# santi-pdp/segan_pytorch

Measured on AMD Instinct MI355X. Metric: 16384-sample waveform chunks/sec (GAN step), higher is better.
Workload: dtype f32

## Files before the change

segan_pytorch_amd/_lib.py:

```python
import ctypes
import os
import re
from ctypes import POINTER, Structure, c_char_p, c_double, c_float, c_int, c_int32, c_int64, c_size_t, c_void_p

_HERE = os.path.dirname(os.path.abspath(__file__))
LIB_PATH = os.environ.get('SEGAN_HIP_LIB') or os.path.join(_HERE, 'libsegan_hip.so')
HEADER_PATH = os.path.join(os.path.dirname(_HERE), 'include', 'segan_hip.h')


class SeganSrc(Structure):
    _fields_ = [('p0', c_void_p), ('p1', c_void_p), ('C0', c_int32), ('C1', c_int32),
                ('scale', c_void_p), ('shift', c_void_p), ('slope', c_void_p)]


_SCALARS = {'int': c_int, 'float': c_float, 'double': c_double, 'size_t': c_size_t,
            'int64_t': c_int64, 'long long': c_int64}


class _Defines(dict):

    def __init__(self, where):
        dict.__init__(self)
        self.where, self.unread = where, {}

    def __missing__(self, name):
        raise RuntimeError('{}: no integer `#define {}` ({})'.format(
            self.where, name, self.unread.get(name, 'not defined')))


def _ctype(text, decl, ret=False):
    tok = [w for w in re.findall(r'\w+|\S', text) if w != 'const']
    if not ret:
        if len(tok) < 2 or not re.match(r'[A-Za-z_]\w*$', tok[-1]):
            raise RuntimeError('unnamed or unreadable argument `{}` in `{}`'.format(text.strip(), decl))
        tok.pop()
    stars = tok.count('*')
    base = tok[:len(tok) - stars]
    if stars and base and '*' not in base:
        if not ret:
            return POINTER(SeganSrc) if tok == ['segan_src', '*'] else c_void_p
        if tok == ['char', '*']:
            return c_char_p
    elif ret and tok == ['void']:
        return None
    elif ' '.join(tok) in _SCALARS:
        return _SCALARS[' '.join(tok)]
    raise RuntimeError('unknown type `{}` in `{}`'.format(text.strip(), decl))


def read_header(text, where='<text>'):
    text = re.sub(r'/\*.*?\*/|//[^\n]*', ' ', text, flags=re.S)
    defines = _Defines(where)
    seen = {}
    for name, val in re.findall(r'^[ \t]*#[ \t]*define[ \t]+(SEGAN_\w+)[ \t]+(\S.*?)[ \t]*$', text, flags=re.M):
        seen.setdefault(name, []).append(val)
    for name, vals in seen.items():
        if len(set(vals)) == 1 and re.match(r'-?(0[xX][0-9a-fA-F]+|[1-9]\d*|0)$', vals[0]):
            defines[name] = int(vals[0], 0)
        else:
            defines.unread[name] = ' / '.join('#define {} {}'.format(name, v) for v in vals)
    text = re.sub(r'^[ \t]*#.*$', '', text, flags=re.M)
    signatures = {}
    for m in re.finditer(r'[^;{}]*\bsegan_\w+\s*\([^;]*(;|$)', text):
        decl = ' '.join(m.group().split())
        d = re.match(r'([\w\s*]+?)\s*\b(segan_\w+)\s*\(([^()]*)\)\s*;$', decl)
        if not d or d.group(2) in signatures:
            raise RuntimeError('{}: cannot read the declaration `{}`'.format(where, decl))
        args = [] if d.group(3).strip() == 'void' else d.group(3).split(',')
        signatures[d.group(2)] = (_ctype(d.group(1), decl, ret=True), [_ctype(a, decl) for a in args])
    return signatures, defines


def _read_header_file():
    if not os.path.exists(HEADER_PATH):
        raise RuntimeError('segan_pytorch_amd: {} not found. The ctypes binding is read from the '
                           'header the library is built against.'.format(HEADER_PATH))
    with open(HEADER_PATH) as f:
        return read_header(f.read(), HEADER_PATH)


SIGNATURES, DEFINES = _read_header_file()

PAD_REFLECT = DEFINES['SEGAN_PAD_REFLECT']
PAD_ZERO = DEFINES['SEGAN_PAD_ZERO']
ACT_NONE = DEFINES['SEGAN_ACT_NONE']
ACT_TANH = DEFINES['SEGAN_ACT_TANH']
ABI_VERSION = DEFINES['SEGAN_ABI_VERSION']

_lib = None


def load():
    global _lib
    if _lib is not None:
        return _lib
    if not os.path.exists(LIB_PATH):
        raise RuntimeError(
            'segan_pytorch_amd: {} not found. Build it with `make` (or '
            '`python -c "import __graft_entry__ as g; g.build()"`) at the repo root. '
            'There is no non-HIP fallback.'.format(LIB_PATH))
    try:
        import torch
        if torch.cuda.is_available():
            torch.cuda.init()
    except ImportError:
        pass
    lib = ctypes.CDLL(LIB_PATH)
    for name, (res, args) in SIGNATURES.items():
        fn = getattr(lib, name)
        fn.restype = res
        fn.argtypes = args
    ver = lib.segan_abi_version()
    if ver != ABI_VERSION:
        raise RuntimeError('libsegan_hip ABI {} != expected {}'.format(ver, ABI_VERSION))
    _lib = lib
    return lib


def check(rc, what=''):
    if rc != 0:
        msg = load().segan_last_error()
        raise RuntimeError('libsegan_hip {} failed ({}): {}'.format(
            what, rc, msg.decode() if msg else '?'))
```

segan_pytorch_amd/csrc/segan_conv.hip:

```cpp
#include "segan_conv_tile.h"


struct TileWork {
  int tile, c0, c1;
  bool partial;
  int piece;
};

struct TileIter {
  int tileA;
  long unit, unit_end;
  int first_tile;
  __device__ __forceinline__ void init(const CorrArgs& a, int nch) {
    tileA = blockIdx.x;
    unit = (long)blockIdx.x * a.sk_units;
    unit_end = min(unit + (long)a.sk_units, a.sk_total);
    first_tile = (int)(unit / nch);
  }
  __device__ __forceinline__ bool next(const CorrArgs& a, int nch, TileWork& w) {
    if (tileA < a.sk_nfull) {
      const int rd = tileA / (int)gridDim.x;
      const int left = a.sk_nfull - rd * (int)gridDim.x;
      w.tile = rd * (int)gridDim.x + xcd_remap(blockIdx.x, left < (int)gridDim.x ? left : (int)gridDim.x);
      w.c0 = 0; w.c1 = nch; w.partial = false; w.piece = 0;
      tileA += gridDim.x;
      return true;
    }
    if (unit < unit_end) {
      const int t = (int)(unit / nch);
      w.c0 = (int)(unit - (long)t * nch);
      w.c1 = min(nch, w.c0 + (int)(unit_end - unit));
      unit += w.c1 - w.c0;
      w.tile = a.sk_nfull + t;
      w.partial = (w.c0 != 0) || (w.c1 != nch);
      w.piece = t - first_tile;
      return true;
    }
    return false;
  }
};

template <int MB, int U, int KC, int NI, int NJ, bool SHIFT, int FMODE = 0, int ZP = -1, int NPT = 32>
__device__ __forceinline__ void corr_mma_chunk(const float* Wl, const float* Il, int RLs,
                                               const int (&aoff)[NI], const int (&boff)[NJ],
                                               const int (&rsh)[NI], f32x16 (&acc)[NI][NJ],
                                               float (&b30)[NJ], int h, const int (&aoffx)[NI],
                                               const int (&boffx)[NJ]) {
  static_assert(FMODE == 0 || (!SHIFT && ZP < 0), "the pair trick of the F form has no row shifts");
  constexpr int NBI = SHIFT ? NI : 1;
  constexpr int CVC = KC / U;
  constexpr bool ZT = ZP >= 0 && CVC >= 2;
  typedef const volatile __attribute__((address_space(3))) float* ldsp;
  auto special = [](int i) { return ZT && (32 * i) / NPT == ZP; };
  auto skipped = [&](int i, int s) { return special(i) && ((2 * s) % U) == 0; };
  float av0[NI], av1[NI], bv0[NBI][NJ], bv1[NBI][NJ];
  auto read_step = [&](int s, float (&av)[NI], float (&bv)[NBI][NJ]) {
    const int kk = 2 * s;
    const int c = kk / U, u = kk % U;
    ldsp wr = (ldsp)(Wl + kk * MB);
    ldsp ir = (ldsp)(Il + c * RLs + u);
#pragma unroll
    for (int i = 0; i < NI; ++i)
      if (!skipped(i, s)) av[i] = wr[aoff[i]];
#pragma unroll
    for (int i = 0; i < NBI; ++i)
#pragma unroll
      for (int j = 0; j < NJ; ++j)
        if (!(SHIFT && skipped(i, s))) bv[i][j] = ir[boff[j] + (SHIFT ? rsh[i] : 0)];
  };
  constexpr int NS = FMODE == 1 ? KC / 2 - 1 : KC / 2;
  auto mma_step = [&](int s, const float (&av)[NI], float (&bv)[NBI][NJ]) {
    if (FMODE == 2 && s == NS - 1) {
#pragma unroll
      for (int j = 0; j < NJ; ++j) bv[0][j] = h ? b30[j] : bv[0][j];
    }
#pragma unroll
    for (int i = 0; i < NI; ++i)
#pragma unroll
      for (int j = 0; j < NJ; ++j)
        if (!skipped(i, s))
          acc[i][j] = __builtin_amdgcn_mfma_f32_32x32x2f32(av[i], bv[SHIFT ? i : 0][j], acc[i][j],
                                                           0, 0, 0);
  };
// ... 920 lines not shown
  SEGAN_REQUIRE(precision_ok(precision), "deconv1d_dgrad: precision must be 0, 1, 3 or 4");
  SEGAN_REQUIRE(stride_ok(S), "deconv1d_dgrad: stride %d not in {1,2,4}", S);
  SEGAN_REQUIRE(K >= 1 && K <= 32, "deconv1d_dgrad: kernel width %d not in [1,32]", K);
  SEGAN_REQUIRE(B > 0 && N > 0 && M > 0 && Ls > 0, "deconv1d_dgrad: bad sizes");
  SEGAN_REQUIRE(M0 >= 0 && M0 <= M, "deconv1d_dgrad: split %d outside [0,%d]", M0, M);
  SEGAN_REQUIRE(dy && wf, "deconv1d_dgrad: NULL pointer");
  SEGAN_REQUIRE(dx0 || dx1, "deconv1d_dgrad: both destinations NULL");
  const int U = 32 / S;
  CorrArgs a = {};
  a.acc_block = acc_block;
  a.in.p0 = dy; a.in.p1 = nullptr; a.in.C0 = N; a.in.C1 = 0;
  a.in.scale = a.in.shift = a.in.slope = nullptr;
  a.wp = (const float*)wf;
  a.bias = nullptr; a.halo = nullptr;
  a.B = B; a.Cv = N * S; a.Ktot = N * 32; a.RP = f_pitch(M); a.Rvalid = M;
  a.Tcols = Ls; a.Ctot = B * Ls;
  a.Lin = S * Ls; a.padL = pad; a.mode = SEGAN_PAD_ZERO; a.roll = 0;
  a.win_start = 0; a.H = U - 1;
  a.NP = 1; a.Nout = 0;
  if (M0 == 0) { a.out0 = dx1; a.OC0 = M; a.out1 = nullptr; a.OC1 = 0; }
  else { a.out0 = dx0; a.OC0 = M0; a.out1 = dx1; a.OC1 = M - M0; }
  a.Lout = Ls; a.act = SEGAN_ACT_NONE;
  a.out0_elems = (size_t)B * a.OC0 * Ls;
  a.out1_elems = (size_t)B * a.OC1 * Ls;
  a.f_pair = f_pair(N, K); a.zphase = -1;
  if (precision) {
    CorrArgs a2 = a;
    const int e = segan_corr_bf2_f(a2, U, wf, precision, scratch, scratch_bytes, (hipStream_t)stream);
    return e;
  }
  set_scratch(a, scratch, scratch_bytes);
  return launch_corr<true, false>(a, U, (hipStream_t)stream);
}

extern "C" int segan_deconv1d_fwd(const segan_src* x, const void* wt, const float* w,
                                  const float* bias, float* y, int B, int M, int N, int Ls, int K,
                                  int S, int pad, int act, int precision, void* scratch,
                                  size_t scratch_bytes, void* stream) {
  const int acc_block = precision == SEGAN_PREC_FP32_BLOCKED;
  if (acc_block) precision = SEGAN_PREC_FP32;
  SEGAN_REQUIRE(precision_ok(precision), "deconv1d_fwd: precision must be 0, 1, 3 or 4");
  SEGAN_REQUIRE(stride_ok(S), "deconv1d_fwd: stride %d not in {1,2,4}", S);
  SEGAN_REQUIRE(K >= 1 && K <= 32, "deconv1d_fwd: kernel width %d not in [1,32]", K);
  SEGAN_REQUIRE(B > 0 && N > 0 && M > 0 && Ls > 0, "deconv1d_fwd: bad sizes");
  SEGAN_REQUIRE(y && (wt || (w && N <= 2)), "deconv1d_fwd: NULL pointer");
  SEGAN_REQUIRE(pad >= 0 && K - 2 * pad - S == (K & 1),
                "deconv1d_fwd: K=%d S=%d pad=%d does not give an output of S*Ls samples", K, S, pad);
  SEGAN_REQUIRE(act == SEGAN_ACT_NONE || act == SEGAN_ACT_TANH, "deconv1d_fwd: bad activation");
  if (int e = check_src(x, M, "deconv1d_fwd")) return e;
  const int U = 32 / S;
  CorrArgs a = {};
  a.acc_block = acc_block;
  a.in = *x;
  a.wp = (const float*)wt;
  a.out0 = y; a.out1 = nullptr; a.bias = bias; a.halo = nullptr;
  a.NP = t_np(N, S); a.Nout = N;
  a.B = B; a.Cv = M; a.Ktot = M * U; a.RP = t_pitch(N, S); a.Rvalid = S * a.NP;
  a.Tcols = Ls; a.Ctot = B * Ls;
  a.Lin = Ls; a.padL = 0; a.mode = SEGAN_PAD_ZERO; a.roll = 0;
  int cmin = 1 << 30, cmax = 0;
  for (int r = 0; r < S; ++r) {
    const int c = (r + pad) / S;
    cmin = c < cmin ? c : cmin;
    cmax = c > cmax ? c : cmax;
  }
  for (int r = 0; r < 4; ++r) a.rowshift[r] = r < S ? (r + pad) / S - cmin : 0;
  a.win_start = cmin - (U - 1);
  a.H = U - 1 + (cmax - cmin);
  a.OC0 = N; a.OC1 = 0; a.Lout = S * Ls; a.act = act;
  a.o_padL = 0; a.o_roll = 0; a.o_padR = 0;
  a.out0_elems = (size_t)B * N * S * Ls;
  a.f_pair = 0; a.zphase = t_zphase(K, S, pad);
  if (w && N <= 2) return segan_launch_tsmall(a, w, K, M, N, S, pad, (hipStream_t)stream);
  if (precision && act == SEGAN_ACT_NONE) {
    CorrArgs a2 = a;
    const int e = segan_corr_bf2_t(a2, U, wt, precision, scratch, scratch_bytes, (hipStream_t)stream);
    return e;
  }
  SEGAN_REQUIRE(precision == 0, "deconv1d_fwd: tanh epilogue only on the fp32 path");
  set_scratch(a, scratch, scratch_bytes);
  return launch_corr<false, true>(a, U, (hipStream_t)stream);
}

extern "C" int segan_conv1d_dgrad(const float* da, const void* wt, const float* w, float* dx,
                                  float* halo, int B, int N, int M, int L, int K, int S, int padL,
                                  int roll, int precision, void* scratch, size_t scratch_bytes,
                                  void* stream) {
  const int acc_block = precision == SEGAN_PREC_FP32_BLOCKED;
  if (acc_block) precision = SEGAN_PREC_FP32;
  SEGAN_REQUIRE(precision_ok(precision), "conv1d_dgrad: precision must be 0, 1, 3 or 4");
  SEGAN_REQUIRE(stride_ok(S), "conv1d_dgrad: stride %d not in {1,2,4}", S);
  SEGAN_REQUIRE(K >= 1 && K <= 32, "conv1d_dgrad: kernel width %d not in [1,32]", K);
  SEGAN_REQUIRE(B > 0 && N > 0 && M > 0 && L > 0 && L % S == 0, "conv1d_dgrad: bad sizes");
  SEGAN_REQUIRE(da && dx && halo && (wt || (w && N <= 2)), "conv1d_dgrad: NULL pointer");
  SEGAN_REQUIRE(roll > -L && roll < L, "conv1d_dgrad: |roll| must be < L");
  const int padR = K - 1 - padL >= 0 ? (K - S - padL > 0 ? K - S - padL : 0) : -1;
  SEGAN_REQUIRE(padL >= 0 && padR >= 0 && padL < L && K - S - padL < L, "conv1d_dgrad: bad padding");
  const int U = 32 / S;
  const int Ls = L / S;
  hipStream_t st = (hipStream_t)stream;
  CorrArgs a = {};
  a.acc_block = acc_block;
  a.in.p0 = da; a.in.p1 = nullptr; a.in.C0 = M; a.in.C1 = 0;
  a.in.scale = a.in.shift = a.in.slope = nullptr;
  a.wp = (const float*)wt;
  a.out0 = dx; a.out1 = nullptr; a.bias = nullptr; a.halo = halo;
  a.NP = t_np(N, S); a.Nout = N;
  a.B = B; a.Cv = M; a.Ktot = M * U; a.RP = t_pitch(N, S); a.Rvalid = S * a.NP;
  a.Tcols = (L + padL + padR - 1) / S + 1;
  a.Ctot = B * a.Tcols;
  a.Lin = Ls; a.padL = 0; a.mode = SEGAN_PAD_ZERO; a.roll = 0;
  for (int r = 0; r < 4; ++r) a.rowshift[r] = 0;
  a.win_start = -(U - 1);
  a.H = U - 1;
  a.OC0 = N; a.OC1 = 0; a.Lout = L; a.act = SEGAN_ACT_NONE;
  a.o_padL = padL; a.o_roll = roll; a.o_padR = padR;
  a.out0_elems = (size_t)B * N * L;
  a.halo_elems = (size_t)B * N * (padL + padR);
  a.f_pair = 0; a.zphase = t_zphase(K, S, 0);
  set_scratch(a, scratch, scratch_bytes);
  int e;
  if (w && N <= 2) {
    e = segan_launch_tsmall(a, w, K, M, N, S, 0, st);
  } else if (precision) {
    CorrArgs a2 = a;
    e = segan_corr_bf2_t(a2, U, wt, precision, scratch, scratch_bytes, st);
  } else {
    e = launch_corr<false, true>(a, U, st);
  }
  if (e) return e;
  if (padL + padR > 0) {
    const int rows = B * N;
    const int per_sample = (padL < L - 1 - padR) ? 1 : 0;
    const long nthreads = per_sample ? (long)rows * (padL + padR) : rows;
    hipLaunchKernelGGL(fold_halo_kernel, dim3((unsigned)((nthreads + 255) / 256)), dim3(256), 0, st,
                       dx, halo, rows, L, padL, padR, roll, per_sample);
    return segan_check_launch("fold_halo_kernel");
  }
  return SEGAN_OK;
}

static bool short_ok(int N, int M, int L, int K, int S, int padL) {
  if (!stride_ok(S) || L % S != 0) return false;
  const int Ls = L / S;
  return (Ls == 4 || Ls == 8 || Ls == 16 || Ls == 32 || Ls == 64) && N % 4 == 0 &&
         M % CS_KC == 0 && K >= 1 && K <= 32 && padL >= 0 && K - 1 - padL >= 0 && padL < L &&
         K - S - padL < L;
}

extern "C" size_t segan_packed_g_bytes(int M, int N, int S) {
  if (!stride_ok(S) || M <= 0 || N <= 0) return 0;
  return (size_t)M * N * 32 * sizeof(float);
}

extern "C" int segan_pack_weights_g(const float* w, float* wg, int M, int N, int K, int S,
                                    void* stream) {
  SEGAN_REQUIRE(w && wg && M > 0 && N > 0, "pack_weights_g: bad arguments");
  SEGAN_REQUIRE(stride_ok(S) && K >= 1 && K <= 32, "pack_weights_g: stride in {1,2,4}, K <= 32");
  const size_t total = (size_t)M * N * 32;
  const int blocks = (int)((total + 255) / 256 > 8192 ? 8192 : (total + 255) / 256);
  hipLaunchKernelGGL(pack_g_kernel, dim3(blocks), dim3(256), 0, (hipStream_t)stream, w, wg, M, N, K,
                     S);
  return segan_check_launch("pack_weights_g");
}

extern "C" int segan_conv1d_dgrad_short(const float* da, const float* wg, float* dx, int B, int N,
                                        int M, int L, int K, int S, int padL, int roll,
                                        void* stream) {
  SEGAN_REQUIRE(da && wg && dx && B > 0, "conv1d_dgrad_short: bad arguments");
  SEGAN_REQUIRE(roll > -L && roll < L, "conv1d_dgrad_short: |roll| must be < L");
  if (!short_ok(N, M, L, K, S, padL)) {
    segan_set_error("conv1d_dgrad_short: geometry not covered (L/S in {4,8,16,32,64}, N %% 4 == 0, "
                    "M %% 16 == 0)");
    return SEGAN_EUNSUPPORTED;
  }
  ShortArgs a;
  a.da = da; a.wg = wg; a.dx = dx;
  a.B = B; a.N = N; a.M = M; a.L = L; a.Ls = L / S; a.padL = padL;
  a.padRw = K - S - padL > 0 ? K - S - padL : 0;
  a.roll = roll;
  a.ncoltiles = ceil_div(B, 128 / a.Ls);
  const size_t lds = 4 * 32 * 65 * sizeof(float);
  const dim3 grid((unsigned)(N / 4 * a.ncoltiles));
  static const bool blocked = [] {
    const char* e = getenv("SEGAN_SHORT_ORDER");
    return !(e && e[0] == '0');
  }();
  a.xr8 = a.xbc = 0;
  if (blocked && (N / 4) % 8 == 0) {
    a.xr8 = N / 4 / 8;
    a.xbc = a.xr8 >= 128 ? 1 : 128 / a.xr8;
  }
  hipStream_t st = (hipStream_t)stream;
  if (S == 4) hipLaunchKernelGGL(conv_dgrad_short_kernel<4>, grid, dim3(256), lds, st, a);
  else if (S == 2) hipLaunchKernelGGL(conv_dgrad_short_kernel<2>, grid, dim3(256), lds, st, a);
  else hipLaunchKernelGGL(conv_dgrad_short_kernel<1>, grid, dim3(256), lds, st, a);
  return segan_check_launch("conv_dgrad_short_kernel");
}
```

segan_pytorch_amd/csrc/segan_conv_edge.hip:

```cpp
#include "segan_conv_shared.h"

template <int S, int N, int PM, int KT>
__global__ __launch_bounds__(256) void tsmall_kernel(const CorrArgs a, const float* __restrict__ w,
                                                     int Krt, int M) {
  const int K = KT ? KT : Krt;
  constexpr int U = 32 / S;
  constexpr int MC = 16;
  constexpr int TW = 256 + U;
  __shared__ float xs[MC][TW + 1];
  const int tid = threadIdx.x;
  const int b = blockIdx.y;
  const int q0 = blockIdx.x * 256;
  const int q = q0 + tid;
  float acc[S][N];
#pragma unroll
  for (int r = 0; r < S; ++r)
#pragma unroll
    for (int n = 0; n < N; ++n) acc[r][n] = 0.0f;

  const int t0 = q0 + a.win_start + tid, t1 = t0 + 256;
  const bool ok0 = t0 >= 0 && t0 < a.Lin, ok1 = tid < U && t1 >= 0 && t1 < a.Lin;
  const int o0 = ok0 ? t0 : 0, o1 = ok1 ? t1 : 0;
  const int bo0 = b * a.in.C0 * a.Lin, bo1 = b * a.in.C1 * a.Lin;
  float pv0[MC], pv1[MC];
  auto load_rows = [&](int mc0) {
#pragma unroll
    for (int mc = 0; mc < MC; ++mc) {
      const int m = mc0 + mc < M ? mc0 + mc : 0;
      const bool seg1 = m >= a.in.C0;
      const float* rowp = seg1 ? a.in.p1 + (size_t)(m - a.in.C0) * a.Lin + bo1
                               : a.in.p0 + (size_t)m * a.Lin + bo0;
      pv0[mc] = rowp[o0];
      pv1[mc] = rowp[o1];
    }
  };
  load_rows(0);
  for (int mc0 = 0; mc0 < M; mc0 += MC) {
#pragma unroll
    for (int mc = 0; mc < MC; ++mc) {
      const bool mok = mc0 + mc < M;
      const ChanXf xf = segan_chan_xf(a.in, mok ? mc0 + mc : 0);
      xs[mc][tid] = (mok && ok0) ? segan_apply_xf(xf, pv0[mc]) : 0.0f;
      if (tid < U) xs[mc][256 + tid] = (mok && ok1) ? segan_apply_xf(xf, pv1[mc]) : 0.0f;
    }
    __syncthreads();
    if (mc0 + MC < M) load_rows(mc0 + MC);
    const int mcn = min(MC, M - mc0);
    for (int mc = 0; mc < mcn; ++mc) {
      float xv[U + 1];
#pragma unroll
      for (int j = 0; j <= U; ++j) xv[j] = xs[mc][tid + j];
      const float* wm = w + (size_t)(mc0 + mc) * N * K;
#pragma unroll
      for (int r = 0; r < S; ++r) {
        const int rho = (r + PM) % S;
        const int cs = (r + PM) / S;
#pragma unroll
        for (int u = 0; u < U; ++u) {
          const int k = S * u + rho;
          if (KT) {
            if (k < KT) {
#pragma unroll
              for (int n = 0; n < N; ++n)
                acc[r][n] = fmaf(wm[n * KT + k], xv[cs + (U - 1) - u], acc[r][n]);
            }
          } else {
            const int kc = k < K ? k : K - 1;
#pragma unroll
            for (int n = 0; n < N; ++n) {
              float wv = wm[n * K + kc];
              wv = k < K ? wv : 0.0f;
              acc[r][n] = fmaf(wv, xv[cs + (U - 1) - u], acc[r][n]);
            }
          }
        }
      }
    }
    __syncthreads();
  }
  if (q >= a.Tcols) return;
#pragma unroll
  for (int r = 0; r < S; ++r)
#pragma unroll
    for (int n = 0; n < N; ++n) {
      float v = acc[r][n] + (a.bias ? a.bias[n] : 0.0f);
      if (a.act == SEGAN_ACT_TANH) v = tanhf(v);
      const int P = S * q + r;
      int ii = P - a.o_padL;
      const size_t rowoff = (size_t)b * N + n;
      if (ii >= 0 && ii < a.Lout) {
        if (a.o_roll != 0) {
          ii -= a.o_roll;
          if (ii < 0) ii += a.Lout;
          if (ii >= a.Lout) ii -= a.Lout;
        }
        a.out0[rowoff * (size_t)a.Lout + ii] = v;
      } else if (a.halo != nullptr) {
        const int hl = a.o_padL + a.o_padR;
        if (ii < 0) a.halo[rowoff * hl + P] = v;
        else if (ii - a.Lout < a.o_padR) a.halo[rowoff * hl + a.o_padL + (ii - a.Lout)] = v;
      }
    }
}

template <int S, int N, int KT>
static int launch_tsmall_snk(const CorrArgs& a, const float* w, int K, int M, int pad,
                             hipStream_t st) {
  dim3 grid(ceil_div(a.Tcols, 256), a.B);
  switch (pad % S) {
    case 0: hipLaunchKernelGGL((tsmall_kernel<S, N, 0, KT>), grid, dim3(256), 0, st, a, w, K, M); break;
    case 1: hipLaunchKernelGGL((tsmall_kernel<S, N, 1 % S, KT>), grid, dim3(256), 0, st, a, w, K, M); break;
    case 2: hipLaunchKernelGGL((tsmall_kernel<S, N, 2 % S, KT>), grid, dim3(256), 0, st, a, w, K, M); break;
    default: hipLaunchKernelGGL((tsmall_kernel<S, N, 3 % S, KT>), grid, dim3(256), 0, st, a, w, K, M); break;
  }
  return segan_check_launch("tsmall_kernel");
}

template <int S, int N>
static int launch_tsmall_sn(const CorrArgs& a, const float* w, int K, int M, int pad,
                            hipStream_t st) {
  if (K == 31) return launch_tsmall_snk<S, N, 31>(a, w, K, M, pad, st);
  return launch_tsmall_snk<S, N, 0>(a, w, K, M, pad, st);
}


template <int N, int PM>
__global__ __launch_bounds__(256) void tsmall4_kernel(const CorrArgs a, const float* __restrict__ w,
                                                      int M) {
  constexpr int S = 4, U = 8, KT = 31, Q = 4;
  constexpr int MC = 8;
  constexpr int TWQ = Q * 256 + 12;
  __shared__ __attribute__((aligned(16))) float xs[MC][TWQ];
  const int tid = threadIdx.x;
  const int b = blockIdx.y;
  const int q0 = blockIdx.x * (Q * 256);
  typedef float f32x2 __attribute__((ext_vector_type(2)));
  f32x2 acc[Q / 2][S][N];
#pragma unroll
  for (int i = 0; i < Q / 2; ++i)
#pragma unroll
    for (int r = 0; r < S; ++r)
#pragma unroll
      for (int n = 0; n < N; ++n) acc[i][r][n] = f32x2{0.0f, 0.0f};
  int so[5];
  unsigned sok = 0u;
#pragma unroll
  for (int i = 0; i < 5; ++i) {
    const int j = tid + 256 * i;
    const int t = q0 + a.win_start + j;
    const bool ok = (i < 4 || tid < 12) && t >= 0 && t < a.Lin;
    so[i] = ok ? t : 0;
    if (ok) sok |= 1u << i;
  }
  const int bo0 = b * a.in.C0 * a.Lin, bo1 = b * a.in.C1 * a.Lin;
  float pv[MC][5];
  auto load_rows = [&](int mc0) {
#pragma unroll
    for (int mc = 0; mc < MC; ++mc) {
      const int m = mc0 + mc < M ? mc0 + mc : 0;
      const bool seg1 = m >= a.in.C0;
      const float* rowp = seg1 ? a.in.p1 + (size_t)(m - a.in.C0) * a.Lin + bo1
                               : a.in.p0 + (size_t)m * a.Lin + bo0;
#pragma unroll
      for (int i = 0; i < 5; ++i) pv[mc][i] = rowp[so[i]];
    }
  };
  load_rows(0);
  for (int mc0 = 0; mc0 < M; mc0 += MC) {
#pragma unroll
    for (int mc = 0; mc < MC; ++mc) {
      const bool mok = mc0 + mc < M;
      const ChanXf xf = segan_chan_xf(a.in, mok ? mc0 + mc : 0);
#pragma unroll
      for (int i = 0; i < 4; ++i)
        xs[mc][tid + 256 * i] = (mok && ((sok >> i) & 1u)) ? segan_apply_xf(xf, pv[mc][i]) : 0.0f;
      if (tid < 12) xs[mc][1024 + tid] = (mok && ((sok >> 4) & 1u)) ? segan_apply_xf(xf, pv[mc][4]) : 0.0f;
    }
    __syncthreads();
    if (mc0 + MC < M) load_rows(mc0 + MC);
    const int mcn = min(MC, M - mc0);
    for (int mc = 0; mc < mcn; ++mc) {
      f32x2 xe[6], xo[5];
#pragma unroll
      for (int i = 0; i < 3; ++i) {
        const f32x4 t4 = *reinterpret_cast<const f32x4*>(&xs[mc][4 * tid + 4 * i]);
        xe[2 * i] = f32x2{t4[0], t4[1]};
        xe[2 * i + 1] = f32x2{t4[2], t4[3]};
      }
#pragma unroll
      for (int i = 0; i < 5; ++i) xo[i] = f32x2{xs[mc][4 * tid + 2 * i + 1], xs[mc][4 * tid + 2 * i + 2]};
      typedef const __attribute__((address_space(4))) float cfl;
      constexpr int NPW = (N * KT + 1) / 2;
      cfl* wm = (cfl*)w + (size_t)(mc0 + mc) * N * KT;
      f32x2 wp[NPW];
#pragma unroll
      for (int p = 0; p < NPW; ++p) {
        const int f0 = 2 * p + 1 < N * KT ? 2 * p : N * KT - 2;
        wp[p] = f32x2{wm[f0], wm[f0 + 1]};
      }
#pragma unroll
      for (int r = 0; r < S; ++r) {
        const int rho = (r + PM) % S, cs = (r + PM) / S;
#pragma unroll
        for (int u = 0; u < U; ++u) {
          const int k = S * u + rho;
          if (k < KT) {
#pragma unroll
            for (int n = 0; n < N; ++n) {
              const int f = n * KT + k;
              const bool last = 2 * (f >> 1) + 1 >= N * KT;
              const int p = f >> 1, h = last ? 1 : (f & 1);
#pragma unroll
              for (int ip = 0; ip < Q / 2; ++ip) {
                const int j = 2 * ip + cs + (U - 1) - u;
                const f32x2 xp = (j & 1) ? xo[j >> 1] : xe[j >> 1];
                if (h)
                  asm("v_pk_fma_f32 %0, %1, %2, %0 op_sel:[1,0,0] op_sel_hi:[1,1,1]"
                      : "+v"(acc[ip][r][n]) : "s"(wp[p]), "v"(xp));
                else
                  asm("v_pk_fma_f32 %0, %1, %2, %0 op_sel:[0,0,0] op_sel_hi:[0,1,1]"
                      : "+v"(acc[ip][r][n]) : "s"(wp[p]), "v"(xp));
              }
            }
          }
        }
      }
    }
    __syncthreads();
  }
#pragma unroll
  for (int n = 0; n < N; ++n) {
    const float bs = a.bias ? a.bias[n] : 0.0f;
    const size_t rowoff = (size_t)b * N + n;
#pragma unroll
    for (int i = 0; i < Q; ++i) {
      const int q = q0 + Q * tid + i;
      if (q >= a.Tcols) continue;
      float v[S];
#pragma unroll
      for (int r = 0; r < S; ++r) {
        v[r] = acc[i >> 1][r][n][i & 1] + bs;
        if (a.act == SEGAN_ACT_TANH) v[r] = tanhf(v[r]);
      }
      const int i0 = S * q - a.o_padL;
      if (a.o_roll == 0 && i0 >= 0 && i0 + 3 < a.Lout && (a.o_padL & 3) == 0) {
        const f32x4 o = {v[0], v[1], v[2], v[3]};
        *reinterpret_cast<f32x4*>(a.out0 + rowoff * (size_t)a.Lout + i0) = o;
        continue;
      }
#pragma unroll
      for (int r = 0; r < S; ++r) {
        const int P = S * q + r;
        int ii = P - a.o_padL;
        if (ii >= 0 && ii < a.Lout) {
          if (a.o_roll != 0) {
            ii -= a.o_roll;
            if (ii < 0) ii += a.Lout;
            if (ii >= a.Lout) ii -= a.Lout;
          }
          a.out0[rowoff * (size_t)a.Lout + ii] = v[r];
        } else if (a.halo != nullptr) {
          const int hl = a.o_padL + a.o_padR;
          if (ii < 0) a.halo[rowoff * hl + P] = v[r];
          else if (ii - a.Lout < a.o_padR) a.halo[rowoff * hl + a.o_padL + (ii - a.Lout)] = v[r];
        }
      }
    }
  }
}

template <int N>
static int launch_tsmall4(const CorrArgs& a, const float* w, int M, int pad, hipStream_t st) {
  dim3 grid(ceil_div(a.Tcols, 1024), a.B);
  switch (pad % 4) {
    case 0: hipLaunchKernelGGL((tsmall4_kernel<N, 0>), grid, dim3(256), 0, st, a, w, M); break;
    case 1: hipLaunchKernelGGL((tsmall4_kernel<N, 1>), grid, dim3(256), 0, st, a, w, M); break;
    case 2: hipLaunchKernelGGL((tsmall4_kernel<N, 2>), grid, dim3(256), 0, st, a, w, M); break;
    default: hipLaunchKernelGGL((tsmall4_kernel<N, 3>), grid, dim3(256), 0, st, a, w, M); break;
  }
  return segan_check_launch("tsmall4_kernel");
}

int segan_launch_tsmall(CorrArgs& a, const float* w, int K, int M, int N, int S, int pad,
                         hipStream_t st) {
  if (int e = segan_src_defaults(&a.in, st, "tsmall")) return e;
  if (S == 4 && K == 31 && a.Tcols >= 1024)
    return N == 1 ? launch_tsmall4<1>(a, w, M, pad, st) : launch_tsmall4<2>(a, w, M, pad, st);
  if (N == 1) {
    if (S == 4) return launch_tsmall_sn<4, 1>(a, w, K, M, pad, st);
    if (S == 2) return launch_tsmall_sn<2, 1>(a, w, K, M, pad, st);
    return launch_tsmall_sn<1, 1>(a, w, K, M, pad, st);
  }
  if (S == 4) return launch_tsmall_sn<4, 2>(a, w, K, M, pad, st);
  if (S == 2) return launch_tsmall_sn<2, 2>(a, w, K, M, pad, st);
  return launch_tsmall_sn<1, 2>(a, w, K, M, pad, st);
}


template <int S, int N, int XW>
__device__ __forceinline__ void fsmall_stage_window(const CorrArgs& a, int b, int t0, int tid,
                                                    float (&xs)[N][XW]) {
  constexpr int NX = (XW + 255) / 256;
  constexpr int BT = 6;
  const float* rows[N];
  ChanXf xf[N];
#pragma unroll
  for (int n = 0; n < N; ++n) {
    rows[n] = segan_src_row(a.in, b, n, a.Lin);
    xf[n] = segan_chan_xf(a.in, n);
  }
#pragma unroll
  for (int g0 = 0; g0 < NX; g0 += BT) {
    float v[N][BT];
    int idx[BT];
#pragma unroll
    for (int i = 0; i < BT; ++i) {
      const int j = tid + 256 * (g0 + i);
      idx[i] = (g0 + i < NX && j < XW) ? segan_hi_index(S * t0 + j, a.Lin, a.padL, a.mode, a.roll) : -1;
#pragma unroll
      for (int n = 0; n < N; ++n) v[n][i] = rows[n][idx[i] >= 0 ? idx[i] : 0];
    }
#pragma unroll
    for (int i = 0; i < BT; ++i) {
      const int j = tid + 256 * (g0 + i);
      if (g0 + i < NX && j < XW) {
#pragma unroll
        for (int n = 0; n < N; ++n) xs[n][j] = idx[i] >= 0 ? segan_apply_xf(xf[n], v[n][i]) : 0.0f;
      }
    }
  }
}

template <int S, int N, int WST>
__device__ __forceinline__ void fsmall_stage_weights(const CorrArgs& a, int m0, int tid, float* ws) {
  constexpr int U = 32 / S;
  constexpr int NW = 64 * N * 32 / 256;
  constexpr int BT = 8;
  static_assert(NW % BT == 0, "weight staging batches");
#pragma unroll
  for (int g0 = 0; g0 < NW; g0 += BT) {
    float v[BT];
#pragma unroll
    for (int i = 0; i < BT; ++i) {
      const int e = tid + 256 * (g0 + i);
      const int ml = e & 63, nk = e >> 6;
      const int n = nk >> 5, k = nk & 31;
      const int row = (n * S + k % S) * U + k / S;
      const int m = m0 + ml;
      v[i] = a.wp[(size_t)row * a.RP + (m < a.RP ? m : 0)];
      v[i] = m < a.RP ? v[i] : 0.0f;
    }
#pragma unroll
    for (int i = 0; i < BT; ++i) {
      const int e = tid + 256 * (g0 + i);
      const int ml = e & 63, nk = e >> 6;
      ws[ml * WST + (nk >> 5) * 32 + (nk & 31)] = v[i];
    }
  }
}

template <int S, int N>
__global__ __launch_bounds__(256) void fsmall_kernel(const CorrArgs a, int M) {
  constexpr int XW = S * 256 + 32;
  constexpr int WST = N * 32 + 4;
  __shared__ __attribute__((aligned(16))) float xs[N][XW];
  __shared__ __attribute__((aligned(16))) float ws[64 * WST];
  const int tid = threadIdx.x;
  const int b = blockIdx.y;
  const int t0 = blockIdx.x * 256;
  fsmall_stage_window<S, N, XW>(a, b, t0, tid, xs);
  const int t = t0 + tid;
  for (int m0 = 0; m0 < M; m0 += 64) {
    fsmall_stage_weights<S, N, WST>(a, m0, tid, ws);
    __syncthreads();
    float xv[N][32];
#pragma unroll
    for (int n = 0; n < N; ++n) {
      if (S == 4) {
#pragma unroll
        for (int i = 0; i < 8; ++i) {
// ... 144 lines not shown
```

segan_pytorch_amd/csrc/segan_conv_shared.h:

```cpp
#pragma once
#include "segan_common.h"
#include <stdlib.h>

#define KCH 64

struct ColTile {
  int col0, b0, t_first, len0;
};

__device__ __forceinline__ ColTile make_coltile(int col0, int Tcols, int NBcols) {
  ColTile t;
  t.col0 = col0;
  t.b0 = col0 / Tcols;
  t.t_first = col0 - t.b0 * Tcols;
  t.len0 = min(Tcols - t.t_first, NBcols);
  return t;
}

__device__ __forceinline__ void lds_pos_decode(const ColTile& ct, int j, int Tcols, int H, int& s,
                                               int& tau) {
  if (j < ct.len0 + H) {
    s = 0;
    tau = ct.t_first + j;
  } else {
// ... 62 lines not shown
  int Ctot;
  int cols_per_split;
  int H, RLw;
  int ls_magic;
  int per_magic;
  int bf_qc;
  int bf_cps;
  int Mp;
  int w2_cps, w2_nch;
  int w2_cpsample;
  int w2_spc;
  int w2_lsshift;
  int w2_pw, w2_nld;
  float* w2_slabs;
};

__device__ __forceinline__ float epi_bias(const float* bias, int base, int rl0, int h) {
  typedef const __attribute__((address_space(4))) float cfloat;
  cfloat* bp = (cfloat*)bias + base;
  const float lo = bp[rl0], hi = bp[rl0 + 4];
  return h ? hi : lo;
}

__device__ __forceinline__ void split3b(float x, __bf16& p1, __bf16& p2, __bf16& p3) {
  p1 = (__bf16)x;
  const float r1 = x - (float)p1;
  p2 = (__bf16)r1;
  const float r2 = r1 - (float)p2;
  p3 = (__bf16)r2;
}

static inline int cur_device() {
  int d = 0;
  (void)hipGetDevice(&d);
  return d & 15;
}

template <typename K>
static void allow_big_lds(K kern, bool (&done)[16]) {
  const int d = cur_device();
  if (!done[d]) {
    (void)hipFuncSetAttribute(reinterpret_cast<const void*>(kern),
                              hipFuncAttributeMaxDynamicSharedMemorySize, 160 * 1024);
    done[d] = true;
  }
}

template <typename K>
static int resident_per_cu(K kern, size_t lds, int (&occ)[16], size_t (&occ_lds)[16], int fallback = 2) {
  const int d = cur_device();
  if (occ[d] == 0 || occ_lds[d] != lds) {
    int nb = 0;
    if (hipOccupancyMaxActiveBlocksPerMultiprocessor(&nb, reinterpret_cast<const void*>(kern), 256,
                                                     lds) != hipSuccess || nb < 1)
      nb = fallback;
    occ[d] = nb > 4 ? 4 : nb;
    occ_lds[d] = lds;
  }
  return occ[d];
}

static inline int f_pitch(int M) { return M <= 64 ? 64 : round_up(M, 128); }
static inline int f_rows(int N) { return round_up(N * 32, KCH); }
static inline int t_pitch(int N, int S) { return S * t_np(N, S); }
static inline int t_rows(int M, int S) { return round_up(M * (32 / S), KCH); }

static inline int f_pair(int N, int K) { return K == 31 && N > 2 && (N & 1) == 0; }
static inline int t_zphase(int K, int S, int pad_t) {
  return (K == 31 && S > 1) ? (((S - 1 - pad_t) % S) + S) % S : -1;
}

static inline bool stride_ok(int S) { return S == 1 || S == 2 || S == 4; }
static inline bool precision_ok(int p) { return p == 0 || p == 1 || p == 3; }
static inline int check_src(const segan_src* s, int C, const char* what) {
  SEGAN_REQUIRE(s != nullptr && s->p0 != nullptr, "%s: source is NULL", what);
  SEGAN_REQUIRE(s->C0 > 0 && s->C1 >= 0 && s->C0 + s->C1 == C,
                "%s: channel segments %d+%d != %d", what, s->C0, s->C1, C);
  SEGAN_REQUIRE(s->C1 == 0 || s->p1 != nullptr, "%s: second segment pointer is NULL", what);
  return SEGAN_OK;
}

int segan_launch_tsmall(CorrArgs& a, const float* w, int K, int M, int N, int S, int pad, hipStream_t st);
int segan_launch_fsmall(CorrArgs& a, int M, int N, int S, hipStream_t st);

void segan_note_corr_launch(int kind, unsigned grid, const CorrArgs& a, int ntiles);
int segan_corr_bf2_f(CorrArgs& a, int U, const void* wp3, int planes, void* scratch,
                     size_t scratch_bytes, hipStream_t st);
int segan_corr_bf2_t(CorrArgs& a, int U, const void* wp3, int planes, void* scratch,
                     size_t scratch_bytes, hipStream_t st);
size_t segan_corr_bf2_scratch_bytes(int B, int Cv, int Tcols, int H, int planes);
int segan_wgrad_bf2(WgradArgs& a, int U, int planes, void* scratch, size_t scratch_bytes, hipStream_t st);
void segan_note_wgrad_launch(int kind, int tiles, int nsplit, int chunks_per_split);
size_t segan_wgrad_bf2_scratch_bytes(int B, int M, int N, int Ls, int S, int planes);
```

segan_pytorch_amd/csrc/segan_pointwise.hip:

```cpp
#include "segan_common.h"

#define PW_THREADS 256

static int pw_nsplit(int B, int C, int L) {
  int ns = ceil_div(2048, C);
  if (ns > B) ns = B;
  long per = (long)B * L / ns;
  while (ns > 1 && per < 2048) {
    ns = (ns + 1) / 2;
    per = (long)B * L / ns;
  }
  return ns < 1 ? 1 : ns;
}

extern "C" int segan_bn_nsplit(int B, int C, int L) {
  if (B <= 0 || C <= 0 || L <= 0) return 0;
  return pw_nsplit(B, C, L);
}

template <int NV>
__device__ __forceinline__ void block_sum(float (&v)[NV], float* sm) {
  const int lane = threadIdx.x & 63, wave = threadIdx.x >> 6;
#pragma unroll
  for (int k = 0; k < NV; ++k) v[k] = warp_sum(v[k]);
  if (lane == 0)
#pragma unroll
    for (int k = 0; k < NV; ++k) sm[wave * NV + k] = v[k];
  __syncthreads();
  if (threadIdx.x == 0) {
#pragma unroll
    for (int k = 0; k < NV; ++k) {
      float s = 0.f;
      for (int w = 0; w < PW_THREADS / 64; ++w) s += sm[w * NV + k];
      v[k] = s;
    }
  }
  __syncthreads();
}

struct ChanRange {
  int c, b_beg, b_end;
};
__device__ __forceinline__ ChanRange chan_range(int B, int nsplit) {
  ChanRange r;
  r.c = blockIdx.x;
  const int per = (B + nsplit - 1) / nsplit;
  r.b_beg = blockIdx.y * per;
  r.b_end = min(B, r.b_beg + per);
  return r;
}

__device__ __forceinline__ void chan_combine(float& n, float& mean, float& m2, float nb, float mb,
                                             float qb) {
  const float tot = n + nb;
  if (tot <= 0.0f) return;
  const float d = mb - mean;
  const float f = nb / tot;
  mean = fmaf(d, f, mean);
  m2 = m2 + qb + d * d * n * f;
  n = tot;
}

__global__ void bn_partial_kernel(const float* __restrict__ x, float* __restrict__ ws, int B, int C,
                                  int L, int nsplit) {
  __shared__ float sm[3 * (PW_THREADS / 64)];
  const ChanRange cr = chan_range(B, nsplit);
  const int nb = cr.b_end - cr.b_beg;
  const float* base = x + ((size_t)cr.b_beg * C + cr.c) * L;
  const size_t sstride = (size_t)C * L;
  const bool vec = (L & 3) == 0 && ((uintptr_t)x & 15) == 0;
  const int Lv = vec ? L >> 2 : L;
  int tr = PW_THREADS;
  while (tr > Lv && tr > 1) tr >>= 1;
  const int rp = PW_THREADS / tr;
  const int t0 = threadIdx.x % tr, r0 = threadIdx.x / tr;
  float K = 0.0f, s1 = 0.0f, s2 = 0.0f, n = 0.0f;
  if (r0 < nb && t0 < Lv) K = base[(size_t)r0 * sstride + (vec ? 4 * t0 : t0)];
  for (int b = r0; b < nb; b += rp) {
    const float* row = base + b * sstride;
    if (vec) {
      for (int t = t0; t < Lv; t += tr) {
        const f32x4 u = *reinterpret_cast<const f32x4*>(row + 4 * t);
#pragma unroll
        for (int e = 0; e < 4; ++e) {
          const float d = u[e] - K;
          s1 += d;
          s2 = fmaf(d, d, s2);
        }
        n += 4.0f;
      }
    } else {
      for (int t = t0; t < Lv; t += tr) {
        const float d = row[t] - K;
        s1 += d;
        s2 = fmaf(d, d, s2);
        n += 1.0f;
      }
    }
  }
  float mean = 0.0f, m2 = 0.0f;
  if (n > 0.0f) {
    const float r = s1 / n;
    mean = K + r;
    m2 = fmaxf(s2 - s1 * r, 0.0f);
  }
#pragma unroll
  for (int o = 32; o > 0; o >>= 1) {
    const float nb2 = __shfl_down(n, o, 64), mb2 = __shfl_down(mean, o, 64), qb2 = __shfl_down(m2, o, 64);
    chan_combine(n, mean, m2, nb2, mb2, qb2);
  }
  const int lane = threadIdx.x & 63, wave = threadIdx.x >> 6;
  if (lane == 0) {
    sm[3 * wave] = n; sm[3 * wave + 1] = mean; sm[3 * wave + 2] = m2;
  }
  __syncthreads();
  if (threadIdx.x == 0) {
    for (int w = 1; w < PW_THREADS / 64; ++w) chan_combine(n, mean, m2, sm[3 * w], sm[3 * w + 1], sm[3 * w + 2]);
    float* w = ws + ((size_t)blockIdx.y * C + cr.c) * 3;
    w[0] = n;
    w[1] = mean;
    w[2] = m2;
  }
}

__device__ __forceinline__ void bn_affine(float gamma, float beta, float mean, float rstd,
                                          float& scale, float& shift) {
  scale = gamma * rstd;
  shift = fmaf(-mean, scale, beta);
}

__global__ void bn_final_kernel(const float* __restrict__ ws, const float* gamma, const float* beta,
                                float eps, float momentum, float* running_mean, float* running_var,
                                float* mean_o, float* rstd_o, float* scale_o, float* shift_o, int C,
                                int nsplit) {
  const int c = blockIdx.x * blockDim.x + threadIdx.x;
  if (c >= C) return;
  double n = 0.0, mean = 0.0, m2 = 0.0;
  for (int s = 0; s < nsplit; ++s) {
    const float* w = ws + ((size_t)s * C + c) * 3;
    const double nb = w[0], mb = w[1], qb = w[2];
    if (nb <= 0.0) continue;
    const double tot = n + nb;
    const double d = mb - mean;
    mean += d * nb / tot;
    m2 += qb + d * d * n * nb / tot;
    n = tot;
  }
  const double var = n > 0 ? m2 / n : 0.0;
  const float rstd = (float)(1.0 / sqrt(var + (double)eps));
  const float g = gamma ? gamma[c] : 1.0f;
  const float bt = beta ? beta[c] : 0.0f;
  float sc, sh;
  bn_affine(g, bt, (float)mean, rstd, sc, sh);
  if (mean_o) mean_o[c] = (float)mean;
  if (rstd_o) rstd_o[c] = rstd;
  if (scale_o) scale_o[c] = sc;
  if (shift_o) shift_o[c] = sh;
  if (running_mean) running_mean[c] = (1.0f - momentum) * running_mean[c] + momentum * (float)mean;
  if (running_var) {
    const double unb = n > 1 ? m2 / (n - 1.0) : var;
    running_var[c] = (1.0f - momentum) * running_var[c] + momentum * (float)unb;
  }
}

extern "C" int segan_bn_stats(const float* x, const float* gamma, const float* beta, float eps,
                              float momentum, float* running_mean, float* running_var, float* mean,
                              float* rstd, float* scale, float* shift, float* ws, int B, int C,
                              int L, void* stream) {
  SEGAN_REQUIRE(x && ws, "bn_stats: NULL pointer");
  SEGAN_REQUIRE(B > 0 && C > 0 && L > 0, "bn_stats: bad sizes");
  hipStream_t st = (hipStream_t)stream;
  const int ns = pw_nsplit(B, C, L);
  hipLaunchKernelGGL(bn_partial_kernel, dim3(C, ns), dim3(PW_THREADS), 0, st, x, ws, B, C, L, ns);
  hipLaunchKernelGGL(bn_final_kernel, dim3(ceil_div(C, 64)), dim3(64), 0, st, ws, gamma, beta, eps,
                     momentum, running_mean, running_var, mean, rstd, scale, shift, C, ns);
  return segan_check_launch("bn_stats");
}

extern "C" int segan_bn_partial(const float* x, float* ws, int B, int C, int L, void* stream) {
  SEGAN_REQUIRE(x && ws, "bn_partial: NULL pointer");
  SEGAN_REQUIRE(B > 0 && C > 0 && L > 0, "bn_partial: bad sizes");
  const int ns = pw_nsplit(B, C, L);
  hipLaunchKernelGGL(bn_partial_kernel, dim3(C, ns), dim3(PW_THREADS), 0, (hipStream_t)stream, x, ws,
                     B, C, L, ns);
  return segan_check_launch("bn_partial");
}

extern "C" int segan_bn_final(const float* ws, int nsplit_total, const float* gamma,
                              const float* beta, float eps, float momentum, float* running_mean,
                              float* running_var, float* mean, float* rstd, float* scale,
                              float* shift, int C, void* stream) {
  SEGAN_REQUIRE(ws && nsplit_total > 0 && C > 0, "bn_final: bad arguments");
  hipLaunchKernelGGL(bn_final_kernel, dim3(ceil_div(C, 64)), dim3(64), 0, (hipStream_t)stream, ws,
                     gamma, beta, eps, momentum, running_mean, running_var, mean, rstd, scale, shift,
                     C, nsplit_total);
  return segan_check_launch("bn_final");
}

__global__ void affine_prelu_kernel(const float* __restrict__ x, const float* scale,
                                    const float* shift, const float* slope, float* __restrict__ y,
                                    size_t total, int C, int L) {
  for (size_t i = blockIdx.x * (size_t)blockDim.x + threadIdx.x; i < total;
       i += (size_t)gridDim.x * blockDim.x) {
    const int c = (int)((i / L) % C);
    float v = x[i];
    v = fmaf(v, scale ? scale[c] : 1.0f, shift ? shift[c] : 0.0f);
    if (slope) v = v > 0.f ? v : v * slope[c];
    y[i] = v;
  }
}

extern "C" int segan_affine_prelu(const float* x, const float* scale, const float* shift,
                                  const float* slope, float* y, int B, int C, int L, void* stream) {
// ... 15 lines not shown
    y[i] = tanhf(fmaf(x[i], scale ? scale[c] : 1.0f, shift ? shift[c] : 0.0f));
  }
}

extern "C" int segan_affine_tanh(const float* x, const float* scale, const float* shift, float* y,
                                 int B, int C, int L, void* stream) {
  SEGAN_REQUIRE(x && y, "affine_tanh: NULL pointer");
  SEGAN_REQUIRE(B > 0 && C > 0 && L > 0, "affine_tanh: bad sizes");
  const size_t total = (size_t)B * C * L;
  const int blocks = (int)((total + 255) / 256 > 4096 ? 4096 : (total + 255) / 256);
  hipLaunchKernelGGL(affine_tanh_kernel, dim3(blocks), dim3(256), 0, (hipStream_t)stream, x, scale,
                     shift, y, total, C, L);
  return segan_check_launch("affine_tanh");
}

__global__ void scale_mask_kernel(const float* __restrict__ x, const float* scale,
                                  const float* __restrict__ mask, float* __restrict__ y,
                                  size_t total, int C, int L) {
  for (size_t i = blockIdx.x * (size_t)blockDim.x + threadIdx.x; i < total;
       i += (size_t)gridDim.x * blockDim.x) {
    const int c = (int)((i / L) % C);
    y[i] = x[i] * (scale ? scale[c] : 1.0f) * mask[i];
  }
}

extern "C" int segan_scale_mask(const float* x, const float* scale, const float* mask, float* y,
                                int B, int C, int L, void* stream) {
  SEGAN_REQUIRE(x && mask && y, "scale_mask: NULL pointer");
  SEGAN_REQUIRE(B > 0 && C > 0 && L > 0, "scale_mask: bad sizes");
  const size_t total = (size_t)B * C * L;
  const int blocks = (int)((total + 255) / 256 > 4096 ? 4096 : (total + 255) / 256);
  hipLaunchKernelGGL(scale_mask_kernel, dim3(blocks), dim3(256), 0, (hipStream_t)stream, x, scale,
                     mask, y, total, C, L);
  return segan_check_launch("scale_mask");
}

__global__ void sum_skip_kernel(const float* __restrict__ x0, const float* slope0,
                                const float* __restrict__ x1, const float* alpha,
                                float* __restrict__ out, size_t total, int C, int L) {
  for (size_t i = blockIdx.x * (size_t)blockDim.x + threadIdx.x; i < total;
       i += (size_t)gridDim.x * blockDim.x) {
    const int c = (int)((i / L) % C);
    float v = x0[i];
    if (slope0) v = v > 0.f ? v : v * slope0[c];
    out[i] = fmaf(alpha[c], x1[i], v);
  }
}

extern "C" int segan_sum_skip(const float* x0, const float* slope0, const float* x1,
                              const float* alpha, float* out, int B, int C, int L, void* stream) {
  SEGAN_REQUIRE(x0 && x1 && alpha && out, "sum_skip: NULL pointer");
  SEGAN_REQUIRE(B > 0 && C > 0 && L > 0, "sum_skip: bad sizes");
  const size_t total = (size_t)B * C * L;
  const int blocks = (int)((total + 255) / 256 > 4096 ? 4096 : (total + 255) / 256);
  hipLaunchKernelGGL(sum_skip_kernel, dim3(blocks), dim3(256), 0, (hipStream_t)stream, x0, slope0,
                     x1, alpha, out, total, C, L);
  return segan_check_launch("sum_skip");
}

struct ActBwdArgs {
  const float* a;
  const float* dh;
  const float* dskip;
  const float* slope;
  const float* alpha;
  const float* mean;
  const float* rstd;
  const float* gamma;
  const float* beta;
  float* da;
  float* ws;
  int B, C, L, nsplit;
  float inv_count;
};

template <int PHASE>
__global__ void act_bwd_kernel(const ActBwdArgs p) {
  __shared__ float sm[16];
  const ChanRange cr = chan_range(p.B, p.nsplit);
  const int c = cr.c;
  const int nb = cr.b_end - cr.b_beg;
  const float sl = p.slope ? p.slope[c] : 1.0f;
  const float al = p.alpha ? p.alpha[c] : 0.0f;
  float mu = 0.f, rs = 1.f, ga = 1.f, be = 0.f, dbeta_m = 0.f, dgamma_m = 0.f, sc = 1.f, sh = 0.f;
  if (PHASE != 0) {
    mu = p.mean[c];
    rs = p.rstd[c];
    ga = p.gamma ? p.gamma[c] : 1.0f;
    be = p.beta ? p.beta[c] : 0.0f;
    bn_affine(ga, be, mu, rs, sc, sh);
  }
  if (PHASE == 2) {
    const float* tot = p.ws + (size_t)p.nsplit * p.C * 4 + (size_t)c * 2;
    dbeta_m = tot[0] * p.inv_count;
    dgamma_m = tot[1] * p.inv_count;
  }
  float r[3] = {0.f, 0.f, 0.f};
  const bool has_skip = p.dskip != nullptr;
  auto elem = [&](float av, float dh, float ds) -> float {
    if (PHASE == 0) {
      float g = dh * (av > 0.f ? 1.0f : sl);
      r[0] += dh * (av > 0.f ? 0.0f : av);
      if (has_skip) {
        g = fmaf(al, ds, g);
        r[1] = fmaf(ds, av, r[1]);
      }
      r[2] += g;
      return g;
    }
    const float xh = (av - mu) * rs;
    const float v = fmaf(av, sc, sh);
    const float g = dh * (v > 0.f ? 1.0f : sl);
    if (PHASE == 1) {
      r[0] += dh * (v > 0.f ? 0.0f : v);
      r[1] += g;
      r[2] = fmaf(g, xh, r[2]);
      return 0.0f;
    }
    const float d = ga * rs * (g - dbeta_m - xh * dgamma_m);
    r[0] += d;
    return d;
  };
  const size_t base = ((size_t)cr.b_beg * p.C + c) * p.L;
  const size_t sstride = (size_t)p.C * p.L;
  const bool vec = (p.L & 3) == 0 &&
                   (((uintptr_t)p.a | (uintptr_t)p.dh | (uintptr_t)p.dskip | (uintptr_t)p.da) & 15) == 0;
  const int Lv = vec ? p.L >> 2 : p.L;
  int tr = PW_THREADS;
  while (tr > Lv && tr > 1) tr >>= 1;
  const int rp = PW_THREADS / tr;
  const int t0 = threadIdx.x % tr, r0 = threadIdx.x / tr;
  const f32x4 z4 = {0.f, 0.f, 0.f, 0.f};
  for (int b = r0; b < nb; b += rp) {
    const size_t ro = base + b * sstride;
    if (vec) {
      for (int t = t0; t < Lv; t += tr) {
        const size_t i = ro + 4 * (size_t)t;
        const f32x4 av = *reinterpret_cast<const f32x4*>(p.a + i);
        const f32x4 dh = p.dh ? *reinterpret_cast<const f32x4*>(p.dh + i) : z4;
        const f32x4 ds = has_skip ? *reinterpret_cast<const f32x4*>(p.dskip + i) : z4;
        f32x4 o;
#pragma unroll
        for (int e = 0; e < 4; ++e) o[e] = elem(av[e], dh[e], ds[e]);
        if (PHASE != 1) *reinterpret_cast<f32x4*>(p.da + i) = o;
      }
    } else {
      for (int t = t0; t < Lv; t += tr) {
        const size_t i = ro + t;
        const float o = elem(p.a[i], p.dh ? p.dh[i] : 0.0f, has_skip ? p.dskip[i] : 0.0f);
        if (PHASE != 1) p.da[i] = o;
      }
    }
  }
  block_sum<3>(r, sm);
  if (threadIdx.x == 0) {
    float* w = p.ws + ((size_t)blockIdx.y * p.C + c) * 4;
    w[0] = r[0];
    w[1] = r[1];
    w[2] = r[2];
  }
}

template <int PHASE>
__global__ void act_bwd_final_kernel(const ActBwdArgs p, float* dslope, float* dalpha,
                                     float* dgamma, float* dbeta, float* dbias) {
  const int c = blockIdx.x * blockDim.x + threadIdx.x;
  if (c >= p.C) return;
  float s0 = 0.f, s1 = 0.f, s2 = 0.f;
  for (int s = 0; s < p.nsplit; ++s) {
    const float* w = p.ws + ((size_t)s * p.C + c) * 4;
    s0 += w[0];
    s1 += w[1];
    s2 += w[2];
  }
  if (PHASE == 0) {
    if (dslope) dslope[c] += s0;
    if (dalpha) dalpha[c] += s1;
    if (dbias) dbias[c] += s2;
  } else if (PHASE == 1) {
    if (dslope) dslope[c] += s0;
    if (dbeta) dbeta[c] += s1;
    if (dgamma) dgamma[c] += s2;
    float* tot = p.ws + (size_t)p.nsplit * p.C * 4 + (size_t)c * 2;
    tot[0] = s1;
    tot[1] = s2;
  } else {
    if (dbias) dbias[c] += s0;
  }
}

extern "C" int segan_act_bwd(const float* a, const float* dh, const float* dskip,
                             const float* slope, const float* alpha, const float* bn_mean,
                             const float* bn_rstd, const float* bn_gamma, const float* bn_beta,
                             float* da, float* dslope, float* dalpha, float* dgamma, float* dbeta,
                             float* dbias, float* ws, int B, int C, int L, void* stream) {
  SEGAN_REQUIRE(a && da && ws, "act_bwd: NULL pointer");
  SEGAN_REQUIRE(dh || dskip, "act_bwd: no incoming gradient");
  SEGAN_REQUIRE(B > 0 && C > 0 && L > 0, "act_bwd: bad sizes");
  SEGAN_REQUIRE((bn_mean == nullptr) == (bn_rstd == nullptr), "act_bwd: mean/rstd must pair");
  SEGAN_REQUIRE(!(dskip && !alpha), "act_bwd: dskip needs alpha");
  SEGAN_REQUIRE(!(bn_mean && dskip), "act_bwd: BN layers have no skip tap");
  hipStream_t st = (hipStream_t)stream;
// ... 486 lines not shown
```

segan_pytorch_amd/csrc/segan_wgrad.hip:

```cpp
#include "segan_conv_tile.h"


template <int TK>
__device__ __forceinline__ int wg_sdiv(int x, int Ls, int magic) {
  return (Ls >= TK) ? (x >= Ls ? 1 : 0) : ((x * magic) >> 16);
}

template <int MB, int NBT>
__global__ __launch_bounds__(256) void wgrad_group_kernel(float* slabs, int nsplit, int gsz) {
  constexpr int NV = (MB / 64) * (NBT / 64) * 4;
  const int tid = threadIdx.x;
  const size_t tile = (size_t)blockIdx.y * gridDim.x + blockIdx.x, ntiles = (size_t)gridDim.x * gridDim.y;
  const int z0 = blockIdx.z * gsz, z1 = min(nsplit, z0 + gsz);
  f32x4 acc[NV];
#pragma unroll
  for (int q = 0; q < NV; ++q) acc[q] = f32x4{0.f, 0.f, 0.f, 0.f};
  for (int z = z0; z < z1; ++z) {
    const f32x4* s4 = reinterpret_cast<const f32x4*>(slabs + ((size_t)z * ntiles + tile) * (MB * NBT));
#pragma unroll
    for (int q = 0; q < NV; ++q) acc[q] += s4[q * 256 + tid];
  }
  f32x4* d4 = reinterpret_cast<f32x4*>(slabs + ((size_t)z0 * ntiles + tile) * (MB * NBT));
#pragma unroll
  for (int q = 0; q < NV; ++q) d4[q * 256 + tid] = acc[q];
}

template <int U, int MB, int NBT, int WM = 2>
__global__ __launch_bounds__(256) void wgrad_reduce_kernel(const WgradArgs a, int nsplit, int zstep = 1) {
  constexpr int S = 32 / U;
  constexpr int WN = 4 / WM;
  constexpr int CVW = NBT / U, NI = MB / (32 * WM), NJ = NBT / (32 * WN);
  const int tid = threadIdx.x;
  const int lane = tid & 63, wave = tid >> 6;
  const int wm = wave / WN, wn = wave % WN;
  const int l31 = lane & 31, h = lane >> 5;
  const int cv0 = blockIdx.x * CVW, m0 = blockIdx.y * MB;
  f32x16 acc[NI][NJ];
#pragma unroll
  for (int i = 0; i < NI; ++i)
#pragma unroll
    for (int j = 0; j < NJ; ++j)
#pragma unroll
      for (int e = 0; e < 16; ++e) acc[i][j][e] = 0.0f;
  for (int z = 0; z < nsplit; z += zstep) {
    const f32x4* s4 = reinterpret_cast<const f32x4*>(
        a.w2_slabs + ((size_t)(z * gridDim.y + blockIdx.y) * gridDim.x + blockIdx.x) * (MB * NBT));
#pragma unroll
    for (int i = 0; i < NI; ++i)
#pragma unroll
      for (int j = 0; j < NJ; ++j)
#pragma unroll
        for (int q = 0; q < 4; ++q) {
          const f32x4 v = s4[((i * NJ + j) * 4 + q) * 256 + tid];
#pragma unroll
          for (int e = 0; e < 4; ++e) acc[i][j][4 * q + e] += v[e];
        }
  }
#pragma unroll
  for (int j = 0; j < NJ; ++j) {
    const int cc = wn * (NBT / WN) + 32 * j + l31;
    const int cv = cv0 + cc / U;
    const int u = cc % U;
    const int n = cv / S, r = cv % S;
    const int k = S * u + r;
    if (cv >= a.Cv || k >= a.K) continue;
#pragma unroll
    for (int i = 0; i < NI; ++i) {
      float old[16];
#pragma unroll
      for (int e = 0; e < 16; ++e) {
        const int m = m0 + wm * (MB / WM) + 32 * i + (e & 3) + 8 * (e >> 2) + 4 * h;
        old[e] = m < a.M ? a.dw[((size_t)m * a.N + n) * a.K + k] : 0.0f;
      }
#pragma unroll
      for (int e = 0; e < 16; ++e) {
        const int m = m0 + wm * (MB / WM) + 32 * i + (e & 3) + 8 * (e >> 2) + 4 * h;
        if (m < a.M) a.dw[((size_t)m * a.N + n) * a.K + k] = old[e] + acc[i][j][e];
      }
    }
  }
}

template <int U, int TK, bool LO_ID, bool HI_ID, int MB, int NBT>
// ... 146 lines not shown
      }
    }
  };

  load_chunk(0);
  store_chunk(0);
  __syncthreads();
  for (int ch = 0; ch < nch; ++ch) {
    const int buf = ch & 1;
    if (ch + 1 < nch) load_chunk(ch + 1);
    const float* Al = Al0 + buf * (MB * AST);
    const float* Bl = Bl0 + buf * (CVW * RLw);
    const int t_first = (split_beg + ch * TK) % Ls;
    int bpos[NJ8][NJ];
#pragma unroll
    for (int j = 0; j < NJ8; ++j) {
      const int k0 = 8 * j + 4 * h;
      const int p = k0 + wg_sdiv<TK>(t_first + k0, Ls, a.ls_magic) * a.H;
#pragma unroll
      for (int jj = 0; jj < NJ; ++jj) bpos[j][jj] = bbase[jj] + p;
    }
    f32x4 af0[NI], af1[NI];
    float bv0[NJ], bv1[NJ];
    auto read_a = [&](int j, f32x4 (&af)[NI]) {
#pragma unroll
      for (int i = 0; i < NI; ++i) af[i] = *reinterpret_cast<const f32x4*>(Al + aoff[i] + 8 * j);
    };
    auto read_b = [&](int s, float (&bv)[NJ]) {
#pragma unroll
      for (int jj = 0; jj < NJ; ++jj) bv[jj] = Bl[bpos[s / 4][jj] + (s & 3)];
    };
    auto mma = [&](const f32x4 (&af)[NI], int e, const float (&bv)[NJ]) {
#pragma unroll
      for (int i = 0; i < NI; ++i)
#pragma unroll
        for (int jj = 0; jj < NJ; ++jj)
          acc[i][jj] = __builtin_amdgcn_mfma_f32_32x32x2f32(af[i][e], bv[jj], acc[i][jj], 0, 0, 0);
    };
    read_a(0, af0);
    read_b(0, bv0);
#define SB __builtin_amdgcn_sched_barrier(0)
#pragma unroll
    for (int j = 0; j < NJ8; j += 2) {
      read_a(j + 1, af1);
      read_b(4 * j + 1, bv1); SB; mma(af0, 0, bv0); SB;
      read_b(4 * j + 2, bv0); SB; mma(af0, 1, bv1); SB;
      read_b(4 * j + 3, bv1); SB; mma(af0, 2, bv0); SB;
      read_b(4 * j + 4, bv0); SB; mma(af0, 3, bv1); SB;
      if (j + 2 < NJ8) read_a(j + 2, af0);
      read_b(4 * j + 5, bv1); SB; mma(af1, 0, bv0); SB;
      read_b(4 * j + 6, bv0); SB; mma(af1, 1, bv1); SB;
      read_b(4 * j + 7, bv1); SB; mma(af1, 2, bv0); SB;
      if (4 * j + 8 < TK / 2) read_b(4 * j + 8, bv0);
      SB; mma(af1, 3, bv1); SB;
    }
#undef SB
    if (ch + 1 < nch) store_chunk(buf ^ 1);
    __syncthreads();
  }

  if (a.w2_slabs) {
    slab_store<NI, NJ>(a.w2_slabs + ((size_t)(blockIdx.z * gridDim.y + blockIdx.y) * gridDim.x +
                                           blockIdx.x) * (MB * NBT), acc, tid);
    return;
  }
#pragma unroll
  for (int j = 0; j < NJ; ++j) {
    const int cc = wn * (NBT / 2) + 32 * j + l31;
    const int cv = cv0 + cc / U;
    const int u = cc % U;
    const int n = cv / S, r = cv % S;
    const int k = S * u + r;
    if (cv >= a.Cv || k >= a.K) continue;
#pragma unroll
    for (int i = 0; i < NI; ++i)
#pragma unroll
      for (int e = 0; e < 16; ++e) {
        const int m = m0 + wm * (MB / 2) + 32 * i + (e & 3) + 8 * (e >> 2) + 4 * h;
        if (m < a.M) atomicAdd(a.dw + ((size_t)m * a.N + n) * a.K + k, acc[i][j][e]);
      }
  }
}

template <int U, int RB, int NN, bool LO_ID, bool HI_ID>
__global__ __launch_bounds__(256, RB >= 4 ? 1 : 2) void wgrad_edge_kernel(const WgradArgs a, int spw) {
  constexpr int S = 32 / U;
  constexpr int MB = RB <= 2 ? 64 : 128;
  constexpr int NIW = MB / 64;
  constexpr int NBLK = RB * NN;
  extern __shared__ __attribute__((aligned(16))) float red[];
  const int tid = threadIdx.x, lane = tid & 63;
  const int wave = __builtin_amdgcn_readfirstlane(tid >> 6);
  const int l31 = lane & 31, h = lane >> 5;
  const int k = S * (l31 % U) + l31 / U;
  const int Ls = a.Ls, Lhi = a.Lhi;
  const int spb = Ls >> 5;
  const int nsteps = a.B * spb;
  constexpr int DEPTH = RB * NN >= 4 ? 1 : 2;
  const int wg_beg = min(nsteps, (int)blockIdx.z * 4 * spw), wg_end = min(nsteps, wg_beg + 4 * spw);
  const int cnt = wg_end - wg_beg > wave ? (wg_end - wg_beg - wave + 3) / 4 : 0;

  f32x16 acc[RB][NN];
#pragma unroll
  for (int i = 0; i < RB; ++i)
#pragma unroll
    for (int j = 0; j < NN; ++j)
#pragma unroll
      for (int e = 0; e < 16; ++e) acc[i][j][e] = 0.0f;

  bool rok[RB];
  ChanXf axf[RB];
#pragma unroll
  for (int i = 0; i < RB; ++i) {
    const int m = 32 * i + l31;
    rok[i] = m < a.M;
    if (!LO_ID) axf[i] = segan_chan_xf(a.lo, rok[i] ? m : 0);
  }
  const int lrow = lane >> 3, lpc = lane & 7;
  int crow[RB][4];
  bool cs1[RB][4];
#pragma unroll
  for (int i = 0; i < RB; ++i)
#pragma unroll
    for (int q = 0; q < 4; ++q) {
      int m = 32 * i + 8 * q + lrow;
      m = m < a.M ? m : 0;
      cs1[i][q] = m >= a.lo.C0;
      crow[i][q] = (cs1[i][q] ? m - a.lo.C0 : m) * Ls;
    }
  const bool rows_full = (a.M & 31) == 0;
  bool hs1[NN];
  int hn[NN];
  ChanXf bxf[NN];
#pragma unroll
  for (int j = 0; j < NN; ++j) {
    const int n = j < a.N ? j : 0;
    hs1[j] = n >= a.hi.C0;
    hn[j] = hs1[j] ? n - a.hi.C0 : n;
    if (!HI_ID) bxf[j] = segan_chan_xf(a.hi, n);
  }

  constexpr int XWIN = 32 * S + 32, XL = (XWIN + 63) / 64;
  constexpr int WLDS = NN * XL * 64 + RB * 1024;
  float* win = red + wave * WLDS;
  float* atile = win + NN * XL * 64;
  struct Regs {
    f32x4 A[RB][4];
    float X[NN][XL];
    unsigned xok;
  };
  auto load = [&](Regs& R, int st) {
    const int b = st / spb;
    const int t0 = (st - b * spb) << 5;
    const float* sb0 = a.lo.p0 + (size_t)b * a.lo.C0 * Ls + t0 + 4 * lpc;
    const float* sb1 = a.lo.p1 + (size_t)b * a.lo.C1 * Ls + t0 + 4 * lpc;
#pragma unroll
    for (int i = 0; i < RB; ++i)
#pragma unroll
      for (int q = 0; q < 4; ++q)
        R.A[i][q] = *reinterpret_cast<const f32x4*>((cs1[i][q] ? sb1 : sb0) + crow[i][q]);
    R.xok = 0u;
    int off[XL];
#pragma unroll
    for (int e = 0; e < XL; ++e) {
      const int pw = lane + 64 * e;
      const int idx = segan_hi_index(S * t0 + pw, Lhi, a.padL, a.mode, a.roll);
      const bool ok = pw < XWIN && idx >= 0;
      if (ok) R.xok |= 1u << e;
      off[e] = ok ? idx : 0;
    }
#pragma unroll
    for (int j = 0; j < NN; ++j) {
      const float* q = hs1[j] ? a.hi.p1 + ((size_t)b * a.hi.C1 + hn[j]) * Lhi
                              : a.hi.p0 + ((size_t)b * a.hi.C0 + hn[j]) * Lhi;
#pragma unroll
      for (int e = 0; e < XL; ++e) R.X[j][e] = q[off[e]];
    }
  };
  auto compute = [&](Regs& R) {
#pragma unroll
    for (int i = 0; i < RB; ++i)
#pragma unroll
      for (int q = 0; q < 4; ++q)
        *reinterpret_cast<f32x4*>(atile + (32 * i + 8 * q + lrow) * 32 + 4 * (lpc ^ lrow)) = R.A[i][q];
    f32x4 Af[RB][4];
#pragma unroll
    for (int i = 0; i < RB; ++i)
#pragma unroll
      for (int q = 0; q < 4; ++q)
        Af[i][q] = *reinterpret_cast<const f32x4*>(atile + (32 * i + l31) * 32 + 4 * ((4 * h + q) ^ (l31 & 7)));
    if (!LO_ID || !rows_full) {
#pragma unroll
      for (int i = 0; i < RB; ++i)
#pragma unroll
        for (int q = 0; q < 4; ++q)
#pragma unroll
          for (int e = 0; e < 4; ++e) {
            float v = Af[i][q][e];
            if (!LO_ID) v = segan_apply_xf(axf[i], v);
            Af[i][q][e] = rok[i] ? v : 0.0f;
          }
    }
#pragma unroll
    for (int j = 0; j < NN; ++j)
#pragma unroll
      for (int e = 0; e < XL; ++e) {
        float v = R.X[j][e];
        if (!HI_ID) v = segan_apply_xf(bxf[j], v);
        win[j * (XL * 64) + lane + 64 * e] = ((R.xok >> e) & 1u) ? v : 0.0f;
      }
    float Bv[NN][16];
#pragma unroll
    for (int j = 0; j < NN; ++j)
#pragma unroll
      for (int s2 = 0; s2 < 16; ++s2) Bv[j][s2] = win[j * (XL * 64) + S * (16 * h + s2) + k];
#pragma unroll
    for (int s2 = 0; s2 < 16; ++s2)
#pragma unroll
      for (int i = 0; i < RB; ++i)
#pragma unroll
        for (int j = 0; j < NN; ++j)
          acc[i][j] = __builtin_amdgcn_mfma_f32_32x32x2f32(Af[i][s2 >> 2][s2 & 3], Bv[j][s2],
                                                           acc[i][j], 0, 0, 0);
  };

  if (cnt > 0) {
    auto stp = [&](int i) { return wg_beg + 4 * min(i, cnt - 1) + wave; };
    if (DEPTH == 1) {
      Regs R0, R1;
      load(R0, stp(0));
      for (int i = 0; i < cnt; i += 2) {
        load(R1, stp(i + 1));
        compute(R0);
        load(R0, stp(i + 2));
        if (i + 1 < cnt) compute(R1);
      }
    } else {
      Regs R0, R1, R2;
      load(R0, stp(0));
      load(R1, stp(1));
      for (int i = 0; i < cnt; i += 3) {
        load(R2, stp(i + 2));
        compute(R0);
        load(R0, stp(i + 3));
        if (i + 1 < cnt) compute(R1);
        load(R1, stp(i + 4));
        if (i + 2 < cnt) compute(R2);
      }
    }
  }

  __syncthreads();
#pragma unroll
  for (int i = 0; i < RB; ++i)
#pragma unroll
    for (int j = 0; j < NN; ++j)
#pragma unroll
      for (int e = 0; e < 16; ++e) red[((wave * NBLK + i * NN + j) * 16 + e) * 64 + lane] = acc[i][j][e];
  __syncthreads();
  const int wm = wave >> 1, wn = wave & 1;
  f32x16 out[NIW][1];
#pragma unroll
  for (int ii = 0; ii < NIW; ++ii) {
    const int rb = wm * NIW + ii;
#pragma unroll
    for (int e = 0; e < 16; ++e) {
      float sum = 0.0f;
      if (rb < RB && wn < NN) {
#pragma unroll
        for (int w = 0; w < 4; ++w) sum += red[((w * NBLK + rb * NN + wn) * 16 + e) * 64 + lane];
      }
      out[ii][0][e] = sum;
    }
  }
  if (a.w2_slabs) {
    slab_store<NIW, 1>(a.w2_slabs + (size_t)blockIdx.z * (MB * 64), out, tid);
    return;
  }
  const int cc = wn * 32 + l31;
  const int cv = cc / U, u = cc % U;
  const int n = cv / S, r = cv % S;
  const int kk = S * u + r;
  if (cv >= a.Cv || kk >= a.K) return;
#pragma unroll
  for (int ii = 0; ii < NIW; ++ii)
#pragma unroll
    for (int e = 0; e < 16; ++e) {
      const int m = wm * (MB / 2) + 32 * ii + (e & 3) + 8 * (e >> 2) + 4 * h;
      if (m < a.M) atomicAdd(a.dw + ((size_t)m * a.N + n) * a.K + kk, out[ii][0][e]);
    }
}

#define WG2_TK 32
#define WG2_NLD 4

template <int U, bool XF, int MB = 128>
__global__ __launch_bounds__(256, 2) void wgrad2_kernel(const WgradArgs a) {
  constexpr int S = 32 / U;
  constexpr int TK = WG2_TK;
  constexpr int NBT = 128;
  constexpr int CVW = NBT / U;
  constexpr int WM = MB >= 64 ? 2 : 1, WN = 4 / WM;
  constexpr int NI = MB / (32 * WM), NJ = NBT / (32 * WN);
  constexpr int NLD = WG2_NLD;
  constexpr int NDMA = MB / 32;
  static_assert(CVW / S == 4, "one real hi channel per wave");
  static_assert(MB == 128 || MB == 64 || MB == 32, "block rows");

  extern __shared__ __attribute__((aligned(16))) float smem[];
  const int RLw = a.RLw;
  float* Al0 = smem;
  float* Bl0 = Al0 + 2 * MB * TK;

  const int tid = threadIdx.x;
  const int lane = tid & 63;
  const int wave = __builtin_amdgcn_readfirstlane(tid >> 6);
  const int wm = wave / WN, wn = wave % WN;
  const int l31 = lane & 31, h = lane >> 5;

  const int cv0 = blockIdx.x * CVW;
  const int m0 = blockIdx.y * MB;
  const int ch_beg = blockIdx.z * a.w2_cps;
  const int ch_end = min(ch_beg + a.w2_cps, a.w2_nch);
  if (ch_beg >= ch_end) return;
  const int Ls = a.Ls;
  const int cpsm = a.w2_cpsample;
  const int spc = a.w2_spc;

  const int b_first = cpsm ? ch_beg / cpsm : ch_beg * spc;
  int tq = cpsm ? ch_beg - b_first * cpsm : 0;
  int brel = 0;

  const long lo_left = (long)(a.B - b_first) * a.M * Ls * 4;
  const __amdgpu_buffer_rsrc_t lor = __builtin_amdgcn_make_buffer_rsrc(
      const_cast<float*>(a.lo.p0) + (size_t)b_first * a.M * Ls, 0,
// ... 304 lines not shown
    hipLaunchKernelGGL((wgrad_reduce_kernel<U, MB, 128, (MB >= 64 ? 2 : 1)>), dim3(ncol, nrow), dim3(256), 0,
                       st, a, nsplit, 1);
    return segan_check_launch("wgrad_reduce_kernel");
  }
  return SEGAN_OK;
}

template <int U, bool XF>
static int launch_wgrad2_rows(WgradArgs& a, hipStream_t st, bool deterministic, float* slabs,
                              size_t slab_floats_avail) {
  if constexpr (U == 16) {
    if (a.M <= 32) return launch_wgrad2<U, XF, 32>(a, st, deterministic, slabs, slab_floats_avail);
    if (a.M <= 64) return launch_wgrad2<U, XF, 64>(a, st, deterministic, slabs, slab_floats_avail);
  }
  return launch_wgrad2<U, XF, 128>(a, st, deterministic, slabs, slab_floats_avail);
}

template <int U, bool LO_ID, bool HI_ID, int MB, int NBT>
static int launch_wgrad_tile(WgradArgs& a, hipStream_t st, float* slabs, size_t slab_floats) {
  constexpr int CVW = NBT / U;
  constexpr int TK = 32;
  int NS;
  if (a.Ls >= TK) NS = (a.Ls % TK == 0) ? 1 : 2;
  else NS = (TK % a.Ls == 0) ? TK / a.Ls : (TK + a.Ls - 2) / a.Ls + 1;
  a.H = U - 1;
  a.RLw = TK + NS * a.H;
  a.RLw += (8 - a.RLw % 32 + 32) % 32;
  if (a.RLw > 256 || a.Ls % 4 != 0) {
    segan_set_error("wgrad: low-rate length %d unsupported for stride %d (needs a multiple of 4, "
                    "and >= %d)", a.Ls, 32 / U, U / 2);
    return SEGAN_EUNSUPPORTED;
  }
  if ((long)a.B * a.M * a.Ls >= (1L << 31) || (long)a.B * a.N * a.Lhi >= (1L << 31)) {
    segan_set_error("wgrad: operand exceeds the 2^31 element indexing limit");
    return SEGAN_EUNSUPPORTED;
  }
  if (int e = segan_src_defaults(&a.lo, st, "wgrad(lo)")) return e;
  if (int e = segan_src_defaults(&a.hi, st, "wgrad(hi)")) return e;
  a.ls_magic = (65536 + a.Ls - 1) / a.Ls;
  a.per_magic = (65536 + a.Ls + a.H - 1) / (a.Ls + a.H);
  const int ncol = ceil_div(a.Cv, CVW);
  const int nrow = ceil_div(a.M, MB);
  const int tiles = ncol * nrow;
  const int chunks = ceil_div(a.Ctot, TK);
  int nsplit = ceil_div(1536, tiles);
  if (nsplit > chunks / 4) nsplit = chunks / 4;
  if (nsplit < 1) nsplit = 1;
  const int chunks_per = ceil_div(chunks, nsplit);
  nsplit = ceil_div(chunks, chunks_per);
  a.cols_per_split = chunks_per * TK;
  const size_t lds = (size_t)(2 * MB * (TK + 4) + 2 * CVW * a.RLw) * sizeof(float);
  auto kern = wgrad_kernel<U, TK, LO_ID, HI_ID, MB, NBT>;
  static bool attr_done[16];
  allow_big_lds(kern, attr_done);
  a.w2_slabs = nullptr;
  if (nsplit == 1) slabs = nullptr;
  if (slabs) {
    if (slab_floats < (size_t)tiles * nsplit * MB * NBT) {
      segan_set_error("wgrad: deterministic mode needs %zu bytes of scratch for the partial tiles",
                      (size_t)tiles * nsplit * MB * NBT * sizeof(float));
      return SEGAN_EINVAL;
    }
    a.w2_slabs = slabs;
  }
  g_last_wgrad[0] = 1; g_last_wgrad[1] = tiles; g_last_wgrad[2] = nsplit; g_last_wgrad[3] = chunks_per;
  g_last_wgrad[4] = 0; g_last_wgrad[5] = 0;
  hipLaunchKernelGGL(kern, dim3(ncol, nrow, nsplit), dim3(256), lds, st, a);
  if (int e = segan_check_launch("wgrad_kernel")) return e;
  if (slabs) {
    int zstep = 1;
    if (nsplit >= 128 && tiles <= 8) {
      zstep = 32;
      hipLaunchKernelGGL((wgrad_group_kernel<MB, NBT>), dim3(ncol, nrow, ceil_div(nsplit, zstep)),
                         dim3(256), 0, st, slabs, nsplit, zstep);
      if (int e = segan_check_launch("wgrad_group_kernel")) return e;
    }
    hipLaunchKernelGGL((wgrad_reduce_kernel<U, MB, NBT>), dim3(ncol, nrow), dim3(256), 0, st, a, nsplit,
                       zstep);
    return segan_check_launch("wgrad_reduce_kernel");
  }
  return SEGAN_OK;
}

static bool wgrad_edge_geometry_ok(const WgradArgs& a, int U) {
  if (a.Cv > 64 / U || a.N > 2) return false;
  if (a.Ls % 32 != 0) return false;
  if (a.M > 128 || (a.M > 64 && a.N > 1)) return false;
  return true;
}

template <int U, int RB, int NN, bool LO_ID, bool HI_ID>
static int launch_wgrad_edge_tile(WgradArgs& a, hipStream_t st, float* slabs, size_t slab_floats) {
  constexpr int MB = RB <= 2 ? 64 : 128;
  if ((long)a.B * a.M * a.Ls >= (1L << 31) || (long)a.B * a.N * a.Lhi >= (1L << 31)) {
    segan_set_error("wgrad: operand exceeds the 2^31 element indexing limit");
    return SEGAN_EUNSUPPORTED;
  }
  if (int e = segan_src_defaults(&a.lo, st, "wgrad(lo)")) return e;
  if (int e = segan_src_defaults(&a.hi, st, "wgrad(hi)")) return e;
  const int nsteps = a.B * (a.Ls / 32);
  constexpr int OCC = RB >= 4 ? 1 : 2;
  int nwg = ceil_div(nsteps, 4 * 8);
  if (nwg > 256 * OCC) nwg = 256 * OCC;
  const int spw = ceil_div(nsteps, 4 * nwg);
  nwg = ceil_div(nsteps, 4 * spw);
  a.w2_slabs = nullptr;
  if (nwg == 1) slabs = nullptr;
  if (slabs) {
    if (slab_floats < (size_t)nwg * MB * 64) {
      segan_set_error("wgrad: deterministic mode needs %zu bytes of scratch for the partial tiles",
                      (size_t)nwg * MB * 64 * sizeof(float));
      return SEGAN_EINVAL;
    }
    a.w2_slabs = slabs;
  }
  g_last_wgrad[0] = 4; g_last_wgrad[1] = 1; g_last_wgrad[2] = nwg; g_last_wgrad[3] = spw;
  g_last_wgrad[4] = 0; g_last_wgrad[5] = 0;
  constexpr int XL = (32 * (32 / U) + 32 + 63) / 64;
  const size_t lds_red = (size_t)4 * RB * NN * 1024 * sizeof(float);
  const size_t lds_win = (size_t)4 * (NN * XL * 64 + RB * 1024) * sizeof(float);
  const size_t lds = lds_red > lds_win ? lds_red : lds_win;
  auto kern = wgrad_edge_kernel<U, RB, NN, LO_ID, HI_ID>;
  static bool attr_done[16];
  allow_big_lds(kern, attr_done);
  hipLaunchKernelGGL(kern, dim3(1, 1, nwg), dim3(256), lds, st, a, spw);
  if (int e = segan_check_launch("wgrad_edge_kernel")) return e;
  if (slabs) {
    int zstep = 1;
    if (nwg >= 128) {
      zstep = 32;
      hipLaunchKernelGGL((wgrad_group_kernel<MB, 64>), dim3(1, 1, ceil_div(nwg, zstep)), dim3(256), 0,
                         st, slabs, nwg, zstep);
      if (int e = segan_check_launch("wgrad_group_kernel")) return e;
    }
    hipLaunchKernelGGL((wgrad_reduce_kernel<U, MB, 64>), dim3(1, 1), dim3(256), 0, st, a, nwg, zstep);
    return segan_check_launch("wgrad_reduce_kernel");
  }
  return SEGAN_OK;
}

template <int U, bool LO_ID, bool HI_ID>
static int launch_wgrad_edge(WgradArgs& a, hipStream_t st, float* slabs, size_t slab_floats) {
  if (a.N == 1) {
    if (a.M <= 32) return launch_wgrad_edge_tile<U, 1, 1, LO_ID, HI_ID>(a, st, slabs, slab_floats);
    if (a.M <= 64) return launch_wgrad_edge_tile<U, 2, 1, LO_ID, HI_ID>(a, st, slabs, slab_floats);
    return launch_wgrad_edge_tile<U, 4, 1, LO_ID, HI_ID>(a, st, slabs, slab_floats);
  }
  if (a.M <= 32) return launch_wgrad_edge_tile<U, 1, 2, LO_ID, HI_ID>(a, st, slabs, slab_floats);
  return launch_wgrad_edge_tile<U, 2, 2, LO_ID, HI_ID>(a, st, slabs, slab_floats);
}

template <int U, bool LO_ID, bool HI_ID>
static int launch_wgrad_x(WgradArgs& a, hipStream_t st, float* slabs, size_t slab_floats) {
  static const bool edge_on = getenv("SEGAN_WGRAD_EDGE") == nullptr || atoi(getenv("SEGAN_WGRAD_EDGE")) != 0;
  if (edge_on && wgrad_edge_geometry_ok(a, U)) return launch_wgrad_edge<U, LO_ID, HI_ID>(a, st, slabs, slab_floats);
  if (a.Cv <= 64 / U) {
    if (a.M <= 64) return launch_wgrad_tile<U, LO_ID, HI_ID, 64, 64>(a, st, slabs, slab_floats);
    return launch_wgrad_tile<U, LO_ID, HI_ID, 128, 64>(a, st, slabs, slab_floats);
  }
  return launch_wgrad_tile<U, LO_ID, HI_ID, 128, 128>(a, st, slabs, slab_floats);
}

template <int U>
static int launch_wgrad_t(WgradArgs& a, hipStream_t st, float* slabs, size_t slab_floats) {
  const bool lo_id = !a.lo.scale && !a.lo.shift && !a.lo.slope;
  const bool hi_id = !a.hi.scale && !a.hi.shift && !a.hi.slope;
  if (lo_id && hi_id) return launch_wgrad_x<U, true, true>(a, st, slabs, slab_floats);
  if (lo_id) return launch_wgrad_x<U, true, false>(a, st, slabs, slab_floats);
  if (hi_id) return launch_wgrad_x<U, false, true>(a, st, slabs, slab_floats);
  return launch_wgrad_x<U, false, false>(a, st, slabs, slab_floats);
}

template <int U>
static int launch_wgrad_fp32(WgradArgs& a, hipStream_t st, bool deterministic, float* scratch,
                             size_t scratch_floats) {
  float* slabs = nullptr;
  size_t slab_floats = 0;
  const size_t lo_floats = (size_t)a.B * a.M * a.Ls;
  const bool lo_plain = !a.lo.scale && !a.lo.shift && !a.lo.slope && a.lo.C1 == 0;
  bool fast = wgrad2_geometry_ok(a, U);
  if (a.mode == SEGAN_PAD_ZERO && a.hi.shift) fast = false;
  if (fast && !wgrad2_middle_ok(a, U)) fast = false;
  if (fast && !lo_plain && (scratch == nullptr || scratch_floats < lo_floats)) fast = false;
  size_t used = (fast && !lo_plain) ? lo_floats : 0;
  if (deterministic) {
    if (scratch == nullptr) {
      segan_set_error("wgrad: deterministic mode needs scratch (segan_wgrad_scratch_bytes)");
      return SEGAN_EINVAL;
    }
    slabs = scratch + used;
    slab_floats = scratch_floats - used;
  }
  if (fast) {
    if (!lo_plain) {
      if (int e = segan_src_defaults(&a.lo, st, "wgrad(lo)")) return e;
      const bool xf = true;
      const long total = (long)lo_floats / 4;
      const unsigned grid = (unsigned)(total / 256 > 8192 ? 8192 : (total + 255) / 256);
      hipLaunchKernelGGL(wgrad_lo_materialize_kernel, dim3(grid), dim3(256), 0, st, a.lo, scratch,
                         a.B, a.M, a.Ls / 4, xf ? 1 : 0);
      if (int e = segan_check_launch("wgrad_lo_materialize_kernel")) return e;
      a.lo.p0 = scratch; a.lo.p1 = nullptr; a.lo.C0 = a.M; a.lo.C1 = 0;
      a.lo.scale = a.lo.shift = a.lo.slope = nullptr;
    }
    const bool hi_xf = a.hi.scale || a.hi.shift || a.hi.slope;
    if (hi_xf) {
      if (int e = segan_src_defaults(&a.hi, st, "wgrad(hi)")) return e;
    }
    const int rc = hi_xf ? launch_wgrad2_rows<U, true>(a, st, deterministic, slabs, slab_floats)
                         : launch_wgrad2_rows<U, false>(a, st, deterministic, slabs, slab_floats);
    if (rc != SEGAN_EUNSUPPORTED) return rc;
  }
  return launch_wgrad_t<U>(a, st, slabs, slab_floats);
}

extern "C" size_t segan_wgrad_scratch_bytes(int B, int M, int N, int Ls, int S, int precision,
                                            int flags) {
  if (B <= 0 || M <= 0 || N <= 0 || Ls <= 0 || !stride_ok(S)) return 0;
  if (precision != SEGAN_PREC_FP32) {
    const int planes = precision == SEGAN_PREC_BF16 ? 1 : 3;
    return segan_wgrad_bf2_scratch_bytes(B, M, N, Ls, S, planes);
  }
  size_t bytes = (size_t)B * M * Ls * sizeof(float);
  if (flags & SEGAN_WGRAD_DETERMINISTIC) {
    const int U = 32 / S;
    const size_t tiles = (size_t)ceil_div(N * S, 128 / U) * ceil_div(M, 128);
    bytes += (tiles > 4096 ? tiles : 4096) * 128 * 128 * sizeof(float);
  }
  return bytes;
}

extern "C" int segan_wgrad(const segan_src* lo, const segan_src* hi, float* dw, int B, int M, int N,
                           int Ls, int K, int S, int padL, int mode, int roll, int precision,
                           int flags, void* scratch, size_t scratch_bytes, void* stream) {
  SEGAN_REQUIRE(precision_ok(precision), "wgrad: bad precision %d", precision);
  SEGAN_REQUIRE(stride_ok(S), "wgrad: stride %d not in {1,2,4}", S);
  SEGAN_REQUIRE(K >= 1 && K <= 32, "wgrad: kernel width %d not in [1,32]", K);
  SEGAN_REQUIRE(B > 0 && N > 0 && M > 0 && Ls > 0, "wgrad: bad sizes");
  SEGAN_REQUIRE(dw != nullptr, "wgrad: dw is NULL");
  SEGAN_REQUIRE(mode == SEGAN_PAD_REFLECT || mode == SEGAN_PAD_ZERO, "wgrad: bad pad mode");
  if (int e = check_src(lo, M, "wgrad(lo)")) return e;
  if (int e = check_src(hi, N, "wgrad(hi)")) return e;
  SEGAN_REQUIRE((((uintptr_t)lo->p0 | (lo->C1 > 0 ? (uintptr_t)lo->p1 : 0)) & 15) == 0,
                "wgrad(lo): segment pointers must be 16-byte aligned");
  const int L = S * Ls;
  SEGAN_REQUIRE(roll > -L && roll < L, "wgrad: |roll| must be < L");
  WgradArgs a = {};
  a.lo = *lo; a.hi = *hi; a.dw = dw;
  a.B = B; a.M = M; a.N = N; a.K = K; a.Ls = Ls; a.Lhi = L;
  a.Cv = N * S; a.padL = padL; a.mode = mode; a.roll = roll;
  a.Ctot = B * Ls;
  hipStream_t st = (hipStream_t)stream;
  if (precision != SEGAN_PREC_FP32) {
    const int planes = precision == SEGAN_PREC_BF16 ? 1 : 3;
    WgradArgs a2 = a;
    return segan_wgrad_bf2(a2, 32 / S, planes, scratch, scratch_bytes, st);
  }
  const bool det = (flags & SEGAN_WGRAD_DETERMINISTIC) != 0;
  float* sc = (float*)scratch;
  const size_t scf = scratch ? scratch_bytes / sizeof(float) : 0;
  switch (S) {
    case 4: return launch_wgrad_fp32<8>(a, st, det, sc, scf);
    case 2: return launch_wgrad_fp32<16>(a, st, det, sc, scf);
    default: return launch_wgrad_fp32<32>(a, st, det, sc, scf);
  }
}
```

segan_pytorch_amd/distributed.py:

```python
import os
import time

import torch
import torch.distributed as dist

from . import ops


def is_dist():
    return dist.is_available() and dist.is_initialized() and dist.get_world_size() > 1


def world_size():
    return dist.get_world_size() if (dist.is_available() and dist.is_initialized()) else 1


def _collectives_on():
    if not (dist.is_available() and dist.is_initialized()):
        return False
    return dist.get_world_size() > 1 or os.environ.get('SEGAN_DP_SINGLE') == '1'


def rank():
    return dist.get_rank() if (dist.is_available() and dist.is_initialized()) else 0
# ... 374 lines not shown
def drop_reducer(optimizer):
    global _active
    r = _reducers.pop(id(optimizer), None)
    if r is not None and _active is r:
        _active = None


def arm(optimizer, passes=1):
    global _active
    if not _collectives_on():
        return
    _active = _reducer(optimizer)
    _active.arm(passes)


def grad_ready(*params):
    if _active is None:
        return
    for p in params:
        if p is not None:
            _active.ready(p)


def allreduce_grads(optimizer):
    global _active
    if not _collectives_on():
        return
    r = _reducer(optimizer)
    if _active is not None and _active is not r:
        _active.armed = False
    r.finish()
    _active = None


def broadcast_params(module, src=0):
    if not _collectives_on():
        return
    with torch.no_grad():
        for t in list(module.parameters()) + list(module.buffers()):
            if _native_cur is not None and t.is_cuda and t.dtype == torch.float32 and t.is_contiguous():
                _native_cur.broadcast(t.data, src)
            else:
                dist.broadcast(t.data, src)
    ops.bump_weights_epoch()


def broadcast_scalar(value, src=0, device=None):
    if not is_dist():
        return float(value)
    if device is None or dist.get_backend() != 'nccl':
        device = torch.device('cpu') if dist.get_backend() != 'nccl' else \
            torch.device('cuda', torch.cuda.current_device())
    t = torch.tensor([float(value)], dtype=torch.float64, device=device)
    dist.broadcast(t, src)
    return float(t.item())


def shard_batch(t, dim=0):
    ws, rk = world_size(), rank()
    if ws <= 1:
        return t
    n = t.shape[dim]
    if n % ws != 0:
        raise ValueError('global batch {} is not divisible by world size {}'.format(n, ws))
    per = n // ws
    return t.narrow(dim, rk * per, per)


def sync_bn_enabled():
    return _collectives_on() and os.environ.get("SEGAN_SYNC_BN", "0") == "1"


def bn_stats_sync(x, gamma, beta, eps, momentum, running_mean, running_var):
    ws = ops.bn_partial(x)
    if _native_cur is not None:
        allp = _native_cur.allgather(ws).view(-1, ws.shape[1], 3)
    else:
        parts = [torch.empty_like(ws) for _ in range(world_size())]
        dist.all_gather(parts, ws)
        allp = torch.cat(parts, 0).contiguous()
    return ops.bn_final(allp, gamma, beta, eps, momentum, running_mean, running_var)


def act_bwd_bn_sync(a, dh, slope, bn, dslope=None, dgamma=None, dbeta=None, dbias=None):
    totals, ws = ops.act_bwd_bn_reduce(a, dh, slope, bn, dslope, dgamma, dbeta)
    if _native_cur is not None:
        _native_cur.allreduce(totals, 1.0)
    else:
        dist.all_reduce(totals, op=dist.ReduceOp.SUM)
    count = float(a.shape[0]) * float(a.shape[2]) * world_size()
    return ops.act_bwd_bn_apply(a, dh, slope, bn, totals, count, dbias, ws)
```

segan_pytorch_amd/functional.py:

```python
import os

import torch

from . import ops
from .ops import ACT_NONE, ACT_TANH, PAD_REFLECT, PAD_ZERO, Src


def grad_buf(p):
    if p.grad is None:
        p.grad = torch.zeros_like(p, memory_format=torch.contiguous_format)
    elif not p.grad.is_contiguous():
        p.grad = p.grad.contiguous()
    return p.grad


def _gb(p, needed=True):
    if p is None or not needed or not p.requires_grad:
        return None
    return grad_buf(p)


def _bn_batch_stats(bn, training):
    return training or bn.running_mean is None or bn.running_var is None


def _bn_train_stats(c, bn, training=True):
    from . import distributed as sdist
    fn = sdist.bn_stats_sync if sdist.sync_bn_enabled() else ops.bn_stats
    track = training and bn.running_mean is not None and bn.running_var is not None
    momentum = 0.0
    if track:
        if bn.num_batches_tracked is not None:
            bn.num_batches_tracked += 1
        if bn.momentum is not None:
            momentum = bn.momentum
        else:
            momentum = 1.0 / float(bn.num_batches_tracked) if bn.num_batches_tracked is not None else 0.0
    return fn(c, bn.weight, bn.bias, bn.eps, momentum, bn.running_mean if track else None,
              bn.running_var if track else None)


def _bn_eval_affine(bn):
    rstd = torch.rsqrt(bn.running_var + bn.eps)
    gamma = bn.weight.detach() if bn.weight is not None else torch.ones_like(rstd)
    beta = bn.bias.detach() if bn.bias is not None else torch.zeros_like(rstd)
    scale = (gamma * rstd).contiguous()
    shift = (beta - bn.running_mean * scale).contiguous()
    return scale, shift, rstd.contiguous()


def _eval_bn_act_bwd(c, bn, scale, shift, rstd, dh, slope, dslope, y_tanh=None, dbias=None):
    if y_tanh is not None:
        g = ops.tanh_bwd(y_tanh, dh, dbias=_gb(bn.bias))
    else:
        v = ops.affine_prelu(c, scale, shift, None)
        g = ops.act_bwd(v, dh, slope=slope, dslope=dslope, dbias=_gb(bn.bias))
    if bn.weight is not None and bn.weight.requires_grad:
        xhat = ops.affine_prelu(c, rstd, (-bn.running_mean * rstd).contiguous(), None)
        grad_buf(bn.weight).add_((g * xhat).sum((0, 2)))
    dc = ops.affine_prelu(g, scale, None, None)
    if dbias is not None:
        ops.act_bwd(dc, dc, dbias=dbias)
    return dc


def _act_bwd_bn(a, dh, slope, bn, dslope, dgamma, dbeta, dbias):
    from . import distributed as sdist
    if sdist.sync_bn_enabled():
        return sdist.act_bwd_bn_sync(a, dh, slope, bn, dslope, dgamma, dbeta, dbias)
    return ops.act_bwd(a, dh, slope=slope, bn=bn, dslope=dslope, dgamma=dgamma, dbeta=dbeta,
                       dbias=dbias)


_WGRAD_OVERLAP = os.environ.get('SEGAN_WGRAD_OVERLAP', '0') == '1'
_side_streams = {}


class _SideStream(object):

    def __init__(self, *tensors):
        flat = []
        for t in tensors:
            if isinstance(t, Src):
                flat.extend((t.t0, t.t1, t.scale, t.shift, t.slope))
            else:
                flat.append(t)
        self.tensors = [t for t in flat if torch.is_tensor(t) and t.is_cuda]
        self.on = _WGRAD_OVERLAP and bool(self.tensors)

    def __enter__(self):
        if not self.on:
            return self
        dev = self.tensors[0].device
        main = torch.cuda.current_stream(dev)
        key = (dev.index, main.cuda_stream)
        side = _side_streams.get(key)
        if side is None:
            side = _side_streams[key] = torch.cuda.Stream(device=dev)
        side.wait_stream(main)
        self.side = side
        self.ctx = torch.cuda.stream(side)
        self.ctx.__enter__()
        return self

    def __exit__(self, *exc):
        if not self.on:
            return False
        self.ctx.__exit__(*exc)
        for t in self.tensors:
            t.record_stream(self.side)
        return False


def _join_side(ref):
    if not _WGRAD_OVERLAP or ref is None or not ref.is_cuda:
        return
    main = torch.cuda.current_stream(ref.device)
    side = _side_streams.get((ref.device.index, main.cuda_stream))
    if side is not None:
        main.wait_stream(side)


def _ready(*mods_or_params):
    from . import distributed as sdist
    if sdist._active is None:
        return
    ps = []
    for m in mods_or_params:
        if m is None:
            continue
        if isinstance(m, torch.nn.Module):
            ps.extend(torch.nn.Module.parameters(m))
        else:
            ps.append(m)
    sdist.grad_ready(*ps)


def _ones(n, ref):
    return torch.ones(n, device=ref.device, dtype=torch.float32)


def _cat(a, b):
    return torch.cat((a.detach().reshape(-1), b.detach().reshape(-1)))


import itertools as _it

_sn_epoch = _it.count(1 << 40)


def _is_sn(mod):
    return hasattr(mod, 'weight_orig')


# ... 381 lines not shown
            head = (hf, y1, a1, y2, a2, y3)
        else:
            if pt == 'conv':
                pc = ops.conv1d_fwd(Src(h), W.get(disc.pool_conv), disc.pool_conv.bias, 1,
                                    pad_mode=PAD_ZERO, padL=0, pack=disc._pool_pack)
                hp, idx = pc.view(B, -1), None
                extra['avg_conv_h'] = hp
            else:
                hp, idx = ops.pool_time_fwd(h, 'max' if pt == 'gmax' else 'avg')
            y3 = ops.linear_fwd(hp, W.get(fc))
            out = ops.bias_prelu_rows(y3, fc.bias, None)
            head = (h, hp, idx, y3)
        ctx.disc = disc
        ctx.rolls = tuple(rolls)
        ctx.x_needs = x.requires_grad or (x1 is not None and x1.requires_grad)
        ctx.split = None if x1 is None else (x.shape[1], x.requires_grad, x1.requires_grad)
        ctx.state = (cs, srcs, bns, head, W)
        disc._last_fwd = (cs, xfs)
        disc._last_extra = extra
        disc._last_head = head
        return out

    @staticmethod
    def backward(ctx, dout):
        disc = ctx.disc
        cs, srcs, bns, head, W = ctx.state
        blocks = list(disc.enc_blocks)
        fc = disc.fc
        dout = dout.contiguous()
        def lin_wgrad(mod, dy, xin):
            if W.needs_grad(mod):
                gw = W.grad_target(mod)
                ops.linear_wgrad(dy, xin, gw)
                W.finish(mod, gw)

        def prelu_bwd(y, lin, act, dact):
            gs = W.grad_target(act) if W.needs_grad(act) else None
            d = ops.bias_prelu_rows_bwd(y, lin.bias, W.get(act), dact, gs, _gb(lin.bias))
            if gs is not None:
                W.finish(act, gs)
            return d

        if disc.pool_type == 'none':
            hf, y1, a1, y2, a2, y3 = head
            dy3 = ops.bias_prelu_rows_bwd(y3, fc[4].bias, None, dout, None, _gb(fc[4].bias))
            lin_wgrad(fc[4], dy3, a2)
            da2 = ops.linear_dgrad(dy3, W.get(fc[4]))
            dy2 = prelu_bwd(y2, fc[2], fc[3], da2)
            lin_wgrad(fc[2], dy2, a1)
            da1 = ops.linear_dgrad(dy2, W.get(fc[2]))
            dy1 = prelu_bwd(y1, fc[0], fc[1], da1)
            lin_wgrad(fc[0], dy1, hf)
            dh = ops.linear_dgrad(dy1, W.get(fc[0])).view(cs[-1].shape)
            _ready(fc)
        else:
            h, hp, idx, y3 = head
            Lh = h.shape[2]
            dy3 = ops.bias_prelu_rows_bwd(y3, fc.bias, None, dout, None, _gb(fc.bias))
            lin_wgrad(fc, dy3, hp)
            dhp = ops.linear_dgrad(dy3, W.get(fc))
            if disc.pool_type == 'conv':
                pcm = disc.pool_conv
                dpc = dhp.view(h.shape[0], 1, Lh)
                if pcm.bias is not None and pcm.bias.requires_grad:
                    ops.act_bwd(dpc, dpc, dbias=grad_buf(pcm.bias))
                if W.needs_grad(pcm):
                    gw = W.grad_target(pcm)
                    ops.wgrad(Src(dpc), Src(h), gw, 1, 1, 0, PAD_ZERO)
                    W.finish(pcm, gw)
                dh = ops.conv1d_dgrad(dpc, W.get(pcm), Lh, 1, padL=0, pack=disc._pool_pack)
                _ready(fc, pcm)
            else:
                dh = ops.pool_time_bwd(dhp, idx, Lh, 'max' if disc.pool_type == 'gmax' else 'avg')
                _ready(fc)
        dx = None
        for l in range(len(blocks) - 1, -1, -1):
            blk = blocks[l]
            w = W.get(blk.conv)
            K, S = blk.kwidth, blk.stride
            bn = bns[l]
            if bn == 'eval':
                raise RuntimeError('Discriminator backward in eval() mode with BatchNorm is not '
                                   'supported; call .train() (the reference never does this)')
            if bn is not None:
                dc = _act_bwd_bn(cs[l], dh, blk.act.weight, bn, _gb(blk.act.weight), _gb(bn[2]),
                                 _gb(bn[3]), _gb(blk.conv.bias))
            else:
                dc = ops.act_bwd(cs[l], dh, slope=blk.act.weight, dslope=_gb(blk.act.weight),
                                 dbias=_gb(blk.conv.bias))
            padL = ops.conv_pad(K, S)[0]
            with _SideStream(dc, srcs[l]):
                if W.needs_grad(blk.conv):
                    gw = W.grad_target(blk.conv)
                    ops.wgrad(Src(dc), srcs[l], gw, K, S, padL, PAD_REFLECT, roll=ctx.rolls[l])
                    W.finish(blk.conv, gw)
                _ready(blk)
            if l > 0:
                dh = ops.conv1d_dgrad(dc, w, srcs[l].L, S, roll=ctx.rolls[l], pack=blk._pack)
            elif ctx.x_needs:
                dx = ops.conv1d_dgrad(dc, w, srcs[l].L, S, roll=ctx.rolls[l], pack=blk._pack)
        _join_side(dout)
        ctx.state = None
        dx1 = None
        if dx is not None and ctx.split is not None:
            c0, need0, need1 = ctx.split
            dx1 = dx[:, c0:].contiguous() if need1 else None
            dx = dx[:, :c0].contiguous() if need0 else None
        return (None, None, dx, dx1) + (None,) * (len(ctx.needs_input_grad) - 4)


class ConvBlockFn(torch.autograd.Function):

    @staticmethod
    def forward(ctx, blk, x, *params):
        x = x.contiguous()
        src = Src(x)
        W = _Weights()
        c = ops.conv1d_fwd(src, W.get(blk.conv), blk.conv.bias, blk.stride, pack=blk._pack)
        bn_saved = None
        scale = shift = None
        if blk.norm is not None:
            bn = blk.norm
            if _bn_batch_stats(bn, blk.training):
                mean, rstd, scale, shift = _bn_train_stats(c, bn, blk.training)
                bn_saved = (mean, rstd, bn.weight, bn.bias)
            else:
                scale, shift, rstd = _bn_eval_affine(bn)
                bn_saved = ('eval', scale, shift, rstd)
        h = ops.affine_prelu(c, scale, shift, blk.act.weight)
        a = c if blk.norm is None else ops.affine_prelu(c, scale, shift, None)
        ctx.blk = blk
        ctx.set_materialize_grads(False)
        ctx.x_needs = x.requires_grad
        ctx.state = (src, c, bn_saved, W)
        return h, a

    @staticmethod
    def backward(ctx, dh, da_lin):
        blk = ctx.blk
        src, c, bn, W = ctx.state
        K, S = blk.kwidth, blk.stride
        w = W.get(blk.conv)
        if dh is None and da_lin is None:
            return (None,) * len(ctx.needs_input_grad)
        dh = dh.contiguous() if dh is not None else None
        if bn is None:
            lin = da_lin.contiguous() if da_lin is not None else None
            dc = ops.act_bwd(c, dh, dskip=lin, slope=blk.act.weight,
                             alpha=_ones(c.shape[1], c) if lin is not None else None,
                             dslope=_gb(blk.act.weight), dbias=_gb(blk.conv.bias))
        else:
            if da_lin is not None or dh is None:
                raise RuntimeError('gradient through the linear output of a normalised '
                                   'GConv1DBlock is unsupported')
            if isinstance(bn[0], str):
                dc = _eval_bn_act_bwd(c, blk.norm, bn[1], bn[2], bn[3], dh, blk.act.weight,
                                      _gb(blk.act.weight), dbias=_gb(blk.conv.bias))
            else:
                dc = _act_bwd_bn(c, dh, blk.act.weight, bn, _gb(blk.act.weight), _gb(bn[2]), _gb(bn[3]),
                                 _gb(blk.conv.bias))
        padL = ops.conv_pad(K, S)[0]
        if W.needs_grad(blk.conv):
            gw = W.grad_target(blk.conv)
            ops.wgrad(Src(dc), src, gw, K, S, padL, PAD_REFLECT)
            W.finish(blk.conv, gw)
        dx = ops.conv1d_dgrad(dc, w, src.L, S, pack=blk._pack) if ctx.x_needs else None
# ... 161 lines not shown
```

segan_pytorch_amd/ops.py:

```python
import ctypes
import operator

import numpy as np
import torch

from . import _lib
from . import layout
from ._lib import ACT_NONE, ACT_TANH, PAD_REFLECT, PAD_ZERO, SeganSrc, check


import os as _os

_D = _lib.DEFINES
PREC_FP32, PREC_BF16, PREC_BF16X3 = _D['SEGAN_PREC_FP32'], _D['SEGAN_PREC_BF16'], _D['SEGAN_PREC_BF16X3']
_PREC_NAMES = {'fp32': PREC_FP32, 'bf16': PREC_BF16, 'bf16x3': PREC_BF16X3}
_precision = _PREC_NAMES[_os.environ.get('SEGAN_PRECISION', 'fp32')]
_EUNSUPPORTED = -3


_deterministic = _os.environ.get('SEGAN_DETERMINISTIC', '0') == '1'


def set_deterministic(on):
    global _deterministic
# ... 307 lines not shown
    if padL is None:
        padL = conv_pad(K, S)[0]
    small = N <= 2
    _chk(w, 'weight', 3)
    pack = pack or WeightPack()
    if not small and not _precision and short_rows_ok(N, M, L, S):
        return conv1d_dgrad_short(da, w, L, S, roll=roll, padL=padL, pack=pack)
    dx = torch.empty((B, N, L), device=da.device, dtype=torch.float32)
    halo = torch.empty((B * N * max(K - 1, 1),), device=da.device, dtype=torch.float32)
    lib = _lib.load()
    if small:
        check(lib.segan_conv1d_dgrad(_ptr(da), None, _ptr(w.detach()), _ptr(dx), _ptr(halo), B, N,
                                     M, L, K, S, padL, roll, PREC_FP32, None, 0, _stream()),
              'conv1d_dgrad')
        return dx
    if _precision:
        keep, sp, sn = _bf_scratch(1, B, N, M, L, K, S, padL, da.device)
        rc = lib.segan_conv1d_dgrad(_ptr(da), _ptr(pack.bf(w, S, 0, 1, _precision)), None, _ptr(dx),
                                    _ptr(halo), B, N, M, L, K, S, padL, roll, _precision, sp, sn,
                                    _stream())
        if rc != _EUNSUPPORTED:
            check(rc, 'conv1d_dgrad')
            return dx
    if short_rows_ok(N, M, L, S):
        return conv1d_dgrad_short(da, w, L, S, roll=roll, padL=padL, pack=pack)
    check(lib.segan_conv1d_dgrad(_ptr(da), _ptr(pack.t(w, S, 0)), None, _ptr(dx), _ptr(halo), B, N,
                                 M, L, K, S, padL, roll, _fp32(), *_scratch(), _stream()),
          'conv1d_dgrad')
    return dx


def conv1d_dgrad_short(da, w, L, S, roll=0, padL=None, pack=None):
    _chk(da, 'da', 3)
    _chk(w, 'weight', 3)
    M, N, K = w.shape
    B = da.shape[0]
    if padL is None:
        padL = conv_pad(K, S)[0]
    dx = torch.empty((B, N, L), device=da.device, dtype=torch.float32)
    pack = pack or WeightPack()
    check(_lib.load().segan_conv1d_dgrad_short(_ptr(da), _ptr(pack.g(w, S)), _ptr(dx), B, N,
                                               M, L, K, S, padL, roll, _stream()),
          'conv1d_dgrad_short')
    return dx


_SHORT_LS = (4, 8, 16, 32, 64)


def short_rows_ok(N, M, L, S):
    return S in (2, 4) and L % S == 0 and (L // S) in _SHORT_LS and N % 4 == 0 and M % 16 == 0


def wgrad(lo, hi, dw, K, S, padL, pad_mode, roll=0):
    _chk(dw, 'dw', 3)
    M, N = lo.C, hi.C
    if tuple(dw.shape) != (M, N, K):
        raise ValueError('wgrad: dw {} != ({}, {}, {})'.format(tuple(dw.shape), M, N, K))
    if lo.B != hi.B or lo.L * S != hi.L:
        raise ValueError('wgrad: lo [{}x{}] / hi [{}x{}] inconsistent for stride {}'.format(
            lo.B, lo.L, hi.B, hi.L, S))
    cl, ch = lo.c_struct(), hi.c_struct()
    lib = _lib.load()
    if _precision != PREC_FP32:
        nbytes = lib.segan_wgrad_scratch_bytes(lo.B, M, N, lo.L, S, _precision, 0)
        scratch = _stream_scratch(nbytes, dw.device)
        rc = lib.segan_wgrad(ctypes.byref(cl), ctypes.byref(ch), _ptr(dw), lo.B, M, N, lo.L, K, S,
                             padL, pad_mode, roll, _precision, 0,
                             ctypes.c_void_p(scratch.data_ptr()) if scratch is not None else None,
                             nbytes if scratch is not None else 0, _stream())
        if rc != -3:
            check(rc, 'wgrad')
            return
    flags = 1 if _deterministic else 0
    lo_plain = lo.t1 is None and lo.scale is None and lo.shift is None and lo.slope is None
    scratch, nbytes = None, 0
    if flags or not lo_plain:
        nbytes = lib.segan_wgrad_scratch_bytes(lo.B, M, N, lo.L, S, PREC_FP32, flags)
        scratch = _stream_scratch(nbytes, dw.device)
    check(lib.segan_wgrad(ctypes.byref(cl), ctypes.byref(ch), _ptr(dw), lo.B, M, N, lo.L, K, S, padL,
                          pad_mode, roll, PREC_FP32, flags,
                          ctypes.c_void_p(scratch.data_ptr()) if scratch is not None else None, nbytes,
                          _stream()), 'wgrad')


def deconv1d_fwd(src, w, bias, S, act=ACT_NONE, pack=None):
    M, N, K = w.shape
    if src.C != M:
        raise ValueError('deconv1d_fwd: input has {} channels, weight expects {}'.format(src.C, M))
    pad = deconv_pad(K, S)
    B, Ls = src.B, src.L
    y = torch.empty((B, N, S * Ls), device=w.device, dtype=torch.float32)
    cs = src.c_struct()
    small = N <= 2
    _chk(w, 'weight', 3)
    pack = pack or WeightPack()
    lib = _lib.load()
    if small:
        check(lib.segan_deconv1d_fwd(ctypes.byref(cs), None, _ptr(w.detach()), _ptr(bias), _ptr(y),
                                     B, M, N, Ls, K, S, pad, act, PREC_FP32, None, 0, _stream()),
              'deconv1d_fwd')
        return y
    if _precision and act == ACT_NONE:
        keep, sp, sn = _bf_scratch(2, B, N, M, S * Ls, K, S, pad, w.device)
        rc = lib.segan_deconv1d_fwd(ctypes.byref(cs), _ptr(pack.bf(w, S, pad, 1, _precision)), None,
                                    _ptr(bias), _ptr(y), B, M, N, Ls, K, S, pad, act, _precision,
                                    sp, sn, _stream())
        if rc != _EUNSUPPORTED:
            check(rc, 'deconv1d_fwd')
            return y
    check(lib.segan_deconv1d_fwd(ctypes.byref(cs), _ptr(pack.t(w, S, pad)), None, _ptr(bias),
                                 _ptr(y), B, M, N, Ls, K, S, pad, act, _fp32(), *_scratch(),
                                 _stream()), 'deconv1d_fwd')
    return y


def deconv1d_dgrad(dy, w, S, M0=0, need0=True, need1=True, pack=None):
    _chk(dy, 'dy', 3)
    M, N, K = w.shape
    B = dy.shape[0]
    if dy.shape[1] != N or dy.shape[2] % S != 0:
        raise ValueError('deconv1d_dgrad: dy {} inconsistent with weight {}'.format(
            tuple(dy.shape), tuple(w.shape)))
    Ls = dy.shape[2] // S
    pad = deconv_pad(K, S)
    dx0 = dx1 = None
    if M0 > 0 and need0:
        dx0 = torch.empty((B, M0, Ls), device=dy.device, dtype=torch.float32)
    if M - M0 > 0 and need1:
        dx1 = torch.empty((B, M - M0, Ls), device=dy.device, dtype=torch.float32)
    if dx0 is None and dx1 is None:
        return None, None
    pack = pack or WeightPack()
    lib = _lib.load()
    if _precision:
        keep, sp, sn = _bf_scratch(3, B, N, M, S * Ls, K, S, pad, dy.device)
        rc = lib.segan_deconv1d_dgrad(_ptr(dy), _ptr(pack.bf(w, S, 0, 0, _precision)), _ptr(dx0),
                                      _ptr(dx1), B, M, M0, N, Ls, K, S, pad, _precision, sp, sn,
                                      _stream())
        if rc != _EUNSUPPORTED:
            check(rc, 'deconv1d_dgrad')
            return dx0, dx1
    check(lib.segan_deconv1d_dgrad(_ptr(dy), _ptr(pack.f(w, S)), _ptr(dx0), _ptr(dx1), B, M, M0, N,
                                   Ls, K, S, pad, _fp32(), *_scratch(), _stream()), 'deconv1d_dgrad')
    return dx0, dx1


def _ws(B, C, L, per_split, extra, device):
    ns = _lib.load().segan_bn_nsplit(B, C, L)
    return torch.empty((per_split * ns * C + extra * C,), device=device, dtype=torch.float32)


def bn_stats(x, gamma, beta, eps, momentum, running_mean, running_var):
    _chk(x, 'x', 3)
    B, C, L = x.shape
    mean = torch.empty(C, device=x.device, dtype=torch.float32)
    rstd = torch.empty_like(mean)
    scale = torch.empty_like(mean)
    shift = torch.empty_like(mean)
    ws = _ws(B, C, L, 3, 0, x.device)
    check(_lib.load().segan_bn_stats(_ptr(x), _ptr(gamma), _ptr(beta), eps, momentum,
                                     _ptr(running_mean), _ptr(running_var), _ptr(mean), _ptr(rstd),
                                     _ptr(scale), _ptr(shift), _ptr(ws), B, C, L, _stream()),
          'bn_stats')
    return mean, rstd, scale, shift

# ... 1539 lines not shown
```

Before: 3558.

## Fuse BN+PReLU backward apply into first discriminator layer wgrad/dgrad edge kernels

For the first discriminator layer (N<=2 input channels, BatchNorm), the backward no longer materialises the activation gradient dc through a separate apply kernel. Instead, only the BN reduction totals are computed, and the per-element BN/PReLU backward is recomputed inside the small-channel wgrad or dgrad kernels as they load their inputs. This removes a full write and re-read of a large activation-gradient tensor plus one kernel launch. In exchange, the conv kernels read two tensors (a and dh) instead of one and do extra arithmetic per element, and they gain template variants.

After: 3578 (median of 6 runs). No clear change (+0.6%).

```diff
diff --git a/include/segan_hip_edge.h b/include/segan_hip_edge.h
--- /dev/null
+++ b/include/segan_hip_edge.h
@@ -0,0 +1,23 @@
+#ifndef SEGAN_HIP_EDGE_H
+#define SEGAN_HIP_EDGE_H
+#include "segan_hip.h"
+
+#ifdef __cplusplus
+extern "C" {
+#endif
+
+int segan_wgrad_edge_bn(const float* a, const float* dh, const float* slope, const float* bn_mean,
+                        const float* bn_rstd, const float* bn_gamma, const float* bn_beta,
+                        const float* totals, double count_total, const segan_src* hi, float* dw,
+                        float* dbias, int B, int M, int N, int Ls, int K, int S, int padL, int mode,
+                        int roll, int flags, void* scratch, size_t scratch_bytes, void* stream);
+int segan_conv1d_dgrad_edge_bn(const float* a, const float* dh, const float* slope,
+                               const float* bn_mean, const float* bn_rstd, const float* bn_gamma,
+                               const float* bn_beta, const float* totals, double count_total,
+                               const float* w, float* dx, float* halo, int B, int N, int M, int L,
+                               int K, int S, int padL, int roll, void* stream);
+
+#ifdef __cplusplus
+}
+#endif
+#endif
diff --git a/segan_pytorch_amd/_lib.py b/segan_pytorch_amd/_lib.py
--- a/segan_pytorch_amd/_lib.py
+++ b/segan_pytorch_amd/_lib.py
@@ -6,6 +6,7 @@
 _HERE = os.path.dirname(os.path.abspath(__file__))
 LIB_PATH = os.environ.get('SEGAN_HIP_LIB') or os.path.join(_HERE, 'libsegan_hip.so')
 HEADER_PATH = os.path.join(os.path.dirname(_HERE), 'include', 'segan_hip.h')
+EDGE_HEADER_PATH = os.path.join(os.path.dirname(_HERE), 'include', 'segan_hip_edge.h')
 
 
 class SeganSrc(Structure):
@@ -71,15 +72,19 @@
     return signatures, defines
 
 
-def _read_header_file():
-    if not os.path.exists(HEADER_PATH):
+def _read_header_file(path=HEADER_PATH):
+    if not os.path.exists(path):
         raise RuntimeError('segan_pytorch_amd: {} not found. The ctypes binding is read from the '
-                           'header the library is built against.'.format(HEADER_PATH))
-    with open(HEADER_PATH) as f:
-        return read_header(f.read(), HEADER_PATH)
+                           'header the library is built against.'.format(path))
+    with open(path) as f:
+        return read_header(f.read(), path)
 
 
 SIGNATURES, DEFINES = _read_header_file()
+EDGE_SIGNATURES = _read_header_file(EDGE_HEADER_PATH)[0]
+if set(EDGE_SIGNATURES) & set(SIGNATURES):
+    raise RuntimeError('{} declares again: {}'.format(
+        EDGE_HEADER_PATH, sorted(set(EDGE_SIGNATURES) & set(SIGNATURES))))
 
 PAD_REFLECT = DEFINES['SEGAN_PAD_REFLECT']
 PAD_ZERO = DEFINES['SEGAN_PAD_ZERO']
@@ -106,7 +111,7 @@
     except ImportError:
         pass
     lib = ctypes.CDLL(LIB_PATH)
-    for name, (res, args) in SIGNATURES.items():
+    for name, (res, args) in list(SIGNATURES.items()) + list(EDGE_SIGNATURES.items()):
         fn = getattr(lib, name)
         fn.restype = res
         fn.argtypes = args
diff --git a/segan_pytorch_amd/csrc/segan_act_bwd.h b/segan_pytorch_amd/csrc/segan_act_bwd.h
--- /dev/null
+++ b/segan_pytorch_amd/csrc/segan_act_bwd.h
@@ -0,0 +1,72 @@
+#pragma once
+#include "segan_common.h"
+#include "../../include/segan_hip_edge.h"
+
+__device__ __forceinline__ void bn_affine(float gamma, float beta, float mean, float rstd,
+                                          float& scale, float& shift) {
+  scale = gamma * rstd;
+  shift = fmaf(-mean, scale, beta);
+}
+
+struct BnBwdCoef {
+  float mu, rs;
+  float sc, sh;
+  float gr;
+  float sl;
+  float dbeta_m;
+  float dgamma_m;
+};
+
+struct BnBwdSrc {
+  const float* dh;
+  const float* mean;
+  const float* rstd;
+  const float* gamma;
+  const float* beta;
+  const float* slope;
+  const float* totals;
+  float inv_count;
+};
+
+__device__ __forceinline__ BnBwdCoef bn_bwd_coef(const float* mean, const float* rstd,
+                                                 const float* gamma, const float* beta,
+                                                 const float* slope, int c) {
+  BnBwdCoef k;
+  k.mu = mean[c];
+  k.rs = rstd[c];
+  const float ga = gamma ? gamma[c] : 1.0f;
+  const float be = beta ? beta[c] : 0.0f;
+  k.sl = slope ? slope[c] : 1.0f;
+  bn_affine(ga, be, k.mu, k.rs, k.sc, k.sh);
+  k.gr = ga * k.rs;
+  k.dbeta_m = 0.0f;
+  k.dgamma_m = 0.0f;
+  return k;
+}
+
+__device__ __forceinline__ BnBwdCoef bn_bwd_coef(const BnBwdSrc& s, int c) {
+  BnBwdCoef k = bn_bwd_coef(s.mean, s.rstd, s.gamma, s.beta, s.slope, c);
+  k.dbeta_m = s.totals[2 * c] * s.inv_count;
+  k.dgamma_m = s.totals[2 * c + 1] * s.inv_count;
+  return k;
+}
+
+__device__ __forceinline__ float bn_prelu_gate(const BnBwdCoef& k, float av, float dh, float& xh,
+                                               float& v) {
+  xh = (av - k.mu) * k.rs;
+  v = fmaf(av, k.sc, k.sh);
+  return dh * (v > 0.f ? 1.0f : k.sl);
+}
+
+__device__ __forceinline__ float bn_prelu_bwd(const BnBwdCoef& k, float av, float dh) {
+  float xh, v;
+  const float g = bn_prelu_gate(k, av, dh, xh, v);
+  return k.gr * fmaf(-xh, k.dgamma_m, g - k.dbeta_m);
+}
+
+__device__ __forceinline__ float prelu_skip_bwd(float av, float dh, float ds, float sl, float al,
+                                                bool has_skip) {
+  float g = dh * (av > 0.f ? 1.0f : sl);
+  if (has_skip) g = fmaf(al, ds, g);
+  return g;
+}
diff --git a/segan_pytorch_amd/csrc/segan_conv.hip b/segan_pytorch_amd/csrc/segan_conv.hip
--- a/segan_pytorch_amd/csrc/segan_conv.hip
+++ b/segan_pytorch_amd/csrc/segan_conv.hip
@@ -1,4 +1,5 @@
 #include "segan_conv_tile.h"
+#include "segan_act_bwd.h"
 
 
 struct TileWork {
@@ -1085,25 +1086,10 @@
   return launch_corr<false, true>(a, U, (hipStream_t)stream);
 }
 
-extern "C" int segan_conv1d_dgrad(const float* da, const void* wt, const float* w, float* dx,
-                                  float* halo, int B, int N, int M, int L, int K, int S, int padL,
-                                  int roll, int precision, void* scratch, size_t scratch_bytes,
-                                  void* stream) {
-  const int acc_block = precision == SEGAN_PREC_FP32_BLOCKED;
-  if (acc_block) precision = SEGAN_PREC_FP32;
-  SEGAN_REQUIRE(precision_ok(precision), "conv1d_dgrad: precision must be 0, 1, 3 or 4");
-  SEGAN_REQUIRE(stride_ok(S), "conv1d_dgrad: stride %d not in {1,2,4}", S);
-  SEGAN_REQUIRE(K >= 1 && K <= 32, "conv1d_dgrad: kernel width %d not in [1,32]", K);
-  SEGAN_REQUIRE(B > 0 && N > 0 && M > 0 && L > 0 && L % S == 0, "conv1d_dgrad: bad sizes");
-  SEGAN_REQUIRE(da && dx && halo && (wt || (w && N <= 2)), "conv1d_dgrad: NULL pointer");
-  SEGAN_REQUIRE(roll > -L && roll < L, "conv1d_dgrad: |roll| must be < L");
-  const int padR = K - 1 - padL >= 0 ? (K - S - padL > 0 ? K - S - padL : 0) : -1;
-  SEGAN_REQUIRE(padL >= 0 && padR >= 0 && padL < L && K - S - padL < L, "conv1d_dgrad: bad padding");
+static void dgrad_fill_args(CorrArgs& a, const float* da, const void* wt, float* dx, float* halo, int B,
+                            int N, int M, int L, int K, int S, int padL, int padR, int roll) {
   const int U = 32 / S;
   const int Ls = L / S;
-  hipStream_t st = (hipStream_t)stream;
-  CorrArgs a = {};
-  a.acc_block = acc_block;
   a.in.p0 = da; a.in.p1 = nullptr; a.in.C0 = M; a.in.C1 = 0;
   a.in.scale = a.in.shift = a.in.slope = nullptr;
   a.wp = (const float*)wt;
@@ -1121,6 +1107,38 @@
   a.out0_elems = (size_t)B * N * L;
   a.halo_elems = (size_t)B * N * (padL + padR);
   a.f_pair = 0; a.zphase = t_zphase(K, S, 0);
+}
+
+static int dgrad_fold_halo(float* dx, const float* halo, int B, int N, int L, int padL, int padR,
+                           int roll, hipStream_t st) {
+  if (padL + padR <= 0) return SEGAN_OK;
+  const int rows = B * N;
+  const int per_sample = (padL < L - 1 - padR) ? 1 : 0;
+  const long nthreads = per_sample ? (long)rows * (padL + padR) : rows;
+  hipLaunchKernelGGL(fold_halo_kernel, dim3((unsigned)((nthreads + 255) / 256)), dim3(256), 0, st,
+                     dx, halo, rows, L, padL, padR, roll, per_sample);
+  return segan_check_launch("fold_halo_kernel");
+}
+
+extern "C" int segan_conv1d_dgrad(const float* da, const void* wt, const float* w, float* dx,
+                                  float* halo, int B, int N, int M, int L, int K, int S, int padL,
+                                  int roll, int precision, void* scratch, size_t scratch_bytes,
+                                  void* stream) {
+  const int acc_block = precision == SEGAN_PREC_FP32_BLOCKED;
+  if (acc_block) precision = SEGAN_PREC_FP32;
+  SEGAN_REQUIRE(precision_ok(precision), "conv1d_dgrad: precision must be 0, 1, 3 or 4");
+  SEGAN_REQUIRE(stride_ok(S), "conv1d_dgrad: stride %d not in {1,2,4}", S);
+  SEGAN_REQUIRE(K >= 1 && K <= 32, "conv1d_dgrad: kernel width %d not in [1,32]", K);
+  SEGAN_REQUIRE(B > 0 && N > 0 && M > 0 && L > 0 && L % S == 0, "conv1d_dgrad: bad sizes");
+  SEGAN_REQUIRE(da && dx && halo && (wt || (w && N <= 2)), "conv1d_dgrad: NULL pointer");
+  SEGAN_REQUIRE(roll > -L && roll < L, "conv1d_dgrad: |roll| must be < L");
+  const int padR = K - 1 - padL >= 0 ? (K - S - padL > 0 ? K - S - padL : 0) : -1;
+  SEGAN_REQUIRE(padL >= 0 && padR >= 0 && padL < L && K - S - padL < L, "conv1d_dgrad: bad padding");
+  const int U = 32 / S;
+  hipStream_t st = (hipStream_t)stream;
+  CorrArgs a = {};
+  a.acc_block = acc_block;
+  dgrad_fill_args(a, da, wt, dx, halo, B, N, M, L, K, S, padL, padR, roll);
   set_scratch(a, scratch, scratch_bytes);
   int e;
   if (w && N <= 2) {
@@ -1132,15 +1150,36 @@
     e = launch_corr<false, true>(a, U, st);
   }
   if (e) return e;
-  if (padL + padR > 0) {
-    const int rows = B * N;
-    const int per_sample = (padL < L - 1 - padR) ? 1 : 0;
-    const long nthreads = per_sample ? (long)rows * (padL + padR) : rows;
-    hipLaunchKernelGGL(fold_halo_kernel, dim3((unsigned)((nthreads + 255) / 256)), dim3(256), 0, st,
-                       dx, halo, rows, L, padL, padR, roll, per_sample);
-    return segan_check_launch("fold_halo_kernel");
-  }
-  return SEGAN_OK;
+  return dgrad_fold_halo(dx, halo, B, N, L, padL, padR, roll, st);
+}
+
+extern "C" int segan_conv1d_dgrad_edge_bn(const float* a, const float* dh, const float* slope,
+                                          const float* bn_mean, const float* bn_rstd,
+                                          const float* bn_gamma, const float* bn_beta,
+                                          const float* totals, double count_total, const float* w,
+                                          float* dx, float* halo, int B, int N, int M, int L, int K,
+                                          int S, int padL, int roll, void* stream) {
+  SEGAN_REQUIRE(stride_ok(S), "conv1d_dgrad_edge_bn: stride %d not in {1,2,4}", S);
+  SEGAN_REQUIRE(K >= 1 && K <= 32, "conv1d_dgrad_edge_bn: kernel width %d not in [1,32]", K);
+  SEGAN_REQUIRE(B > 0 && N > 0 && M > 0 && L > 0 && L % S == 0, "conv1d_dgrad_edge_bn: bad sizes");
+  SEGAN_REQUIRE(a && dh && bn_mean && bn_rstd && totals && w && dx && halo,
+                "conv1d_dgrad_edge_bn: NULL pointer");
+  SEGAN_REQUIRE(count_total >= (double)B * (L / S), "conv1d_dgrad_edge_bn: bad element count");
+  SEGAN_REQUIRE(roll > -L && roll < L, "conv1d_dgrad_edge_bn: |roll| must be < L");
+  const int padR = K - 1 - padL >= 0 ? (K - S - padL > 0 ? K - S - padL : 0) : -1;
+  SEGAN_REQUIRE(padL >= 0 && padR >= 0 && padL < L && K - S - padL < L, "conv1d_dgrad_edge_bn: bad padding");
+  if (N > 2 || (L / S) % 32 != 0 || M > 128) {
+    segan_set_error("conv1d_dgrad_edge_bn: not an edge geometry (N <= 2, (L/S) %% 32 == 0, M <= 128)");
+    return SEGAN_EUNSUPPORTED;
+  }
+  hipStream_t st = (hipStream_t)stream;
+  CorrArgs c = {};
+  dgrad_fill_args(c, a, nullptr, dx, halo, B, N, M, L, K, S, padL, padR, roll);
+  BnBwdSrc bn;
+  bn.dh = dh; bn.mean = bn_mean; bn.rstd = bn_rstd; bn.gamma = bn_gamma; bn.beta = bn_beta;
+  bn.slope = slope; bn.totals = totals; bn.inv_count = (float)(1.0 / count_total);
+  if (int e = segan_launch_tsmall_bn(c, w, K, M, N, S, bn, st)) return e;
+  return dgrad_fold_halo(dx, halo, B, N, L, padL, padR, roll, st);
 }
 
 static bool short_ok(int N, int M, int L, int K, int S, int padL) {
diff --git a/segan_pytorch_amd/csrc/segan_conv_edge.hip b/segan_pytorch_amd/csrc/segan_conv_edge.hip
--- a/segan_pytorch_amd/csrc/segan_conv_edge.hip
+++ b/segan_pytorch_amd/csrc/segan_conv_edge.hip
@@ -1,8 +1,9 @@
 #include "segan_conv_shared.h"
-
-template <int S, int N, int PM, int KT>
+#include "segan_act_bwd.h"
+
+template <int S, int N, int PM, int KT, bool BN = false>
 __global__ __launch_bounds__(256) void tsmall_kernel(const CorrArgs a, const float* __restrict__ w,
-                                                     int Krt, int M) {
+                                                     int Krt, int M, const BnBwdSrc bn) {
   const int K = KT ? KT : Krt;
   constexpr int U = 32 / S;
   constexpr int MC = 16;
@@ -23,6 +24,7 @@
   const int o0 = ok0 ? t0 : 0, o1 = ok1 ? t1 : 0;
   const int bo0 = b * a.in.C0 * a.Lin, bo1 = b * a.in.C1 * a.Lin;
   float pv0[MC], pv1[MC];
+  float pd0[BN ? MC : 1], pd1[BN ? MC : 1];
   auto load_rows = [&](int mc0) {
 #pragma unroll
     for (int mc = 0; mc < MC; ++mc) {
@@ -32,6 +34,11 @@
                                : a.in.p0 + (size_t)m * a.Lin + bo0;
       pv0[mc] = rowp[o0];
       pv1[mc] = rowp[o1];
+      if (BN) {
+        const float* rowd = bn.dh + (size_t)m * a.Lin + bo0;
+        pd0[mc] = rowd[o0];
+        pd1[mc] = rowd[o1];
+      }
     }
   };
   load_rows(0);
@@ -39,6 +46,12 @@
 #pragma unroll
     for (int mc = 0; mc < MC; ++mc) {
       const bool mok = mc0 + mc < M;
+      if (BN) {
+        const BnBwdCoef kc = bn_bwd_coef(bn, mok ? mc0 + mc : 0);
+        xs[mc][tid] = (mok && ok0) ? bn_prelu_bwd(kc, pv0[mc], pd0[mc]) : 0.0f;
+        if (tid < U) xs[mc][256 + tid] = (mok && ok1) ? bn_prelu_bwd(kc, pv1[mc], pd1[mc]) : 0.0f;
+        continue;
+      }
       const ChanXf xf = segan_chan_xf(a.in, mok ? mc0 + mc : 0);
       xs[mc][tid] = (mok && ok0) ? segan_apply_xf(xf, pv0[mc]) : 0.0f;
       if (tid < U) xs[mc][256 + tid] = (mok && ok1) ? segan_apply_xf(xf, pv1[mc]) : 0.0f;
@@ -108,10 +121,10 @@
                              hipStream_t st) {
   dim3 grid(ceil_div(a.Tcols, 256), a.B);
   switch (pad % S) {
-    case 0: hipLaunchKernelGGL((tsmall_kernel<S, N, 0, KT>), grid, dim3(256), 0, st, a, w, K, M); break;
-    case 1: hipLaunchKernelGGL((tsmall_kernel<S, N, 1 % S, KT>), grid, dim3(256), 0, st, a, w, K, M); break;
-    case 2: hipLaunchKernelGGL((tsmall_kernel<S, N, 2 % S, KT>), grid, dim3(256), 0, st, a, w, K, M); break;
-    default: hipLaunchKernelGGL((tsmall_kernel<S, N, 3 % S, KT>), grid, dim3(256), 0, st, a, w, K, M); break;
+    case 0: hipLaunchKernelGGL((tsmall_kernel<S, N, 0, KT>), grid, dim3(256), 0, st, a, w, K, M, BnBwdSrc{}); break;
+    case 1: hipLaunchKernelGGL((tsmall_kernel<S, N, 1 % S, KT>), grid, dim3(256), 0, st, a, w, K, M, BnBwdSrc{}); break;
+    case 2: hipLaunchKernelGGL((tsmall_kernel<S, N, 2 % S, KT>), grid, dim3(256), 0, st, a, w, K, M, BnBwdSrc{}); break;
+    default: hipLaunchKernelGGL((tsmall_kernel<S, N, 3 % S, KT>), grid, dim3(256), 0, st, a, w, K, M, BnBwdSrc{}); break;
   }
   return segan_check_launch("tsmall_kernel");
 }
@@ -124,9 +137,9 @@
 }
 
 
-template <int N, int PM>
+template <int N, int PM, bool BN = false>
 __global__ __launch_bounds__(256) void tsmall4_kernel(const CorrArgs a, const float* __restrict__ w,
-                                                      int M) {
+                                                      int M, const BnBwdSrc bn) {
   constexpr int S = 4, U = 8, KT = 31, Q = 4;
   constexpr int MC = 8;
   constexpr int TWQ = Q * 256 + 12;
@@ -154,6 +167,7 @@
   }
   const int bo0 = b * a.in.C0 * a.Lin, bo1 = b * a.in.C1 * a.Lin;
   float pv[MC][5];
+  float pd[BN ? MC : 1][5];
   auto load_rows = [&](int mc0) {
 #pragma unroll
     for (int mc = 0; mc < MC; ++mc) {
@@ -163,6 +177,11 @@
                                : a.in.p0 + (size_t)m * a.Lin + bo0;
 #pragma unroll
       for (int i = 0; i < 5; ++i) pv[mc][i] = rowp[so[i]];
+      if (BN) {
+        const float* rowd = bn.dh + (size_t)m * a.Lin + bo0;
+#pragma unroll
+        for (int i = 0; i < 5; ++i) pd[mc][i] = rowd[so[i]];
+      }
     }
   };
   load_rows(0);
@@ -170,6 +189,14 @@
 #pragma unroll
     for (int mc = 0; mc < MC; ++mc) {
       const bool mok = mc0 + mc < M;
+      if (BN) {
+        const BnBwdCoef kc = bn_bwd_coef(bn, mok ? mc0 + mc : 0);
+#pragma unroll
+        for (int i = 0; i < 4; ++i)
+          xs[mc][tid + 256 * i] = (mok && ((sok >> i) & 1u)) ? bn_prelu_bwd(kc, pv[mc][i], pd[mc][i]) : 0.0f;
+        if (tid < 12) xs[mc][1024 + tid] = (mok && ((sok >> 4) & 1u)) ? bn_prelu_bwd(kc, pv[mc][4], pd[mc][4]) : 0.0f;
+        continue;
+      }
       const ChanXf xf = segan_chan_xf(a.in, mok ? mc0 + mc : 0);
 #pragma unroll
       for (int i = 0; i < 4; ++i)
@@ -273,10 +300,10 @@
 static int launch_tsmall4(const CorrArgs& a, const float* w, int M, int pad, hipStream_t st) {
   dim3 grid(ceil_div(a.Tcols, 1024), a.B);
   switch (pad % 4) {
-    case 0: hipLaunchKernelGGL((tsmall4_kernel<N, 0>), grid, dim3(256), 0, st, a, w, M); break;
-    case 1: hipLaunchKernelGGL((tsmall4_kernel<N, 1>), grid, dim3(256), 0, st, a, w, M); break;
-    case 2: hipLaunchKernelGGL((tsmall4_kernel<N, 2>), grid, dim3(256), 0, st, a, w, M); break;
-    default: hipLaunchKernelGGL((tsmall4_kernel<N, 3>), grid, dim3(256), 0, st, a, w, M); break;
+    case 0: hipLaunchKernelGGL((tsmall4_kernel<N, 0>), grid, dim3(256), 0, st, a, w, M, BnBwdSrc{}); break;
+    case 1: hipLaunchKernelGGL((tsmall4_kernel<N, 1>), grid, dim3(256), 0, st, a, w, M, BnBwdSrc{}); break;
+    case 2: hipLaunchKernelGGL((tsmall4_kernel<N, 2>), grid, dim3(256), 0, st, a, w, M, BnBwdSrc{}); break;
+    default: hipLaunchKernelGGL((tsmall4_kernel<N, 3>), grid, dim3(256), 0, st, a, w, M, BnBwdSrc{}); break;
   }
   return segan_check_launch("tsmall4_kernel");
 }
@@ -296,6 +323,32 @@
   return launch_tsmall_sn<1, 2>(a, w, K, M, pad, st);
 }
 
+template <int S, int N>
+static int launch_tsmall_bn_sn(const CorrArgs& a, const float* w, int K, int M, const BnBwdSrc& bn,
+                               hipStream_t st) {
+  dim3 grid(ceil_div(a.Tcols, 256), a.B);
+  if (K == 31) hipLaunchKernelGGL((tsmall_kernel<S, N, 0, 31, true>), grid, dim3(256), 0, st, a, w, K, M, bn);
+  else hipLaunchKernelGGL((tsmall_kernel<S, N, 0, 0, true>), grid, dim3(256), 0, st, a, w, K, M, bn);
+  return segan_check_launch("tsmall_kernel");
+}
+
+int segan_launch_tsmall_bn(CorrArgs& a, const float* w, int K, int M, int N, int S, const BnBwdSrc& bn,
+                           hipStream_t st) {
+  if (S == 4 && K == 31 && a.Tcols >= 1024) {
+    dim3 grid(ceil_div(a.Tcols, 1024), a.B);
+    if (N == 1) hipLaunchKernelGGL((tsmall4_kernel<1, 0, true>), grid, dim3(256), 0, st, a, w, M, bn);
+    else hipLaunchKernelGGL((tsmall4_kernel<2, 0, true>), grid, dim3(256), 0, st, a, w, M, bn);
+    return segan_check_launch("tsmall4_kernel");
+  }
+  if (N == 1) {
+    if (S == 4) return launch_tsmall_bn_sn<4, 1>(a, w, K, M, bn, st);
+    if (S == 2) return launch_tsmall_bn_sn<2, 1>(a, w, K, M, bn, st);
+    return launch_tsmall_bn_sn<1, 1>(a, w, K, M, bn, st);
+  }
+  if (S == 4) return launch_tsmall_bn_sn<4, 2>(a, w, K, M, bn, st);
+  if (S == 2) return launch_tsmall_bn_sn<2, 2>(a, w, K, M, bn, st);
+  return launch_tsmall_bn_sn<1, 2>(a, w, K, M, bn, st);
+}
 
 template <int S, int N, int XW>
 __device__ __forceinline__ void fsmall_stage_window(const CorrArgs& a, int b, int t0, int tid,
diff --git a/segan_pytorch_amd/csrc/segan_conv_shared.h b/segan_pytorch_amd/csrc/segan_conv_shared.h
--- a/segan_pytorch_amd/csrc/segan_conv_shared.h
+++ b/segan_pytorch_amd/csrc/segan_conv_shared.h
@@ -168,6 +168,9 @@
 
 int segan_launch_tsmall(CorrArgs& a, const float* w, int K, int M, int N, int S, int pad, hipStream_t st);
 int segan_launch_fsmall(CorrArgs& a, int M, int N, int S, hipStream_t st);
+struct BnBwdSrc;
+int segan_launch_tsmall_bn(CorrArgs& a, const float* w, int K, int M, int N, int S, const BnBwdSrc& bn,
+                           hipStream_t st);
 
 void segan_note_corr_launch(int kind, unsigned grid, const CorrArgs& a, int ntiles);
 int segan_corr_bf2_f(CorrArgs& a, int U, const void* wp3, int planes, void* scratch,
diff --git a/segan_pytorch_amd/csrc/segan_pointwise.hip b/segan_pytorch_amd/csrc/segan_pointwise.hip
--- a/segan_pytorch_amd/csrc/segan_pointwise.hip
+++ b/segan_pytorch_amd/csrc/segan_pointwise.hip
@@ -1,4 +1,5 @@
 #include "segan_common.h"
+#include "segan_act_bwd.h"
 
 #define PW_THREADS 256
 
@@ -123,12 +124,6 @@
   }
 }
 
-__device__ __forceinline__ void bn_affine(float gamma, float beta, float mean, float rstd,
-                                          float& scale, float& shift) {
-  scale = gamma * rstd;
-  shift = fmaf(-mean, scale, beta);
-}
-
 __global__ void bn_final_kernel(const float* __restrict__ ws, const float* gamma, const float* beta,
                                 float eps, float momentum, float* running_mean, float* running_var,
                                 float* mean_o, float* rstd_o, float* scale_o, float* shift_o, int C,
@@ -310,42 +305,32 @@
   const int nb = cr.b_end - cr.b_beg;
   const float sl = p.slope ? p.slope[c] : 1.0f;
   const float al = p.alpha ? p.alpha[c] : 0.0f;
-  float mu = 0.f, rs = 1.f, ga = 1.f, be = 0.f, dbeta_m = 0.f, dgamma_m = 0.f, sc = 1.f, sh = 0.f;
-  if (PHASE != 0) {
-    mu = p.mean[c];
-    rs = p.rstd[c];
-    ga = p.gamma ? p.gamma[c] : 1.0f;
-    be = p.beta ? p.beta[c] : 0.0f;
-    bn_affine(ga, be, mu, rs, sc, sh);
-  }
+  BnBwdCoef k = {};
+  if (PHASE != 0) k = bn_bwd_coef(p.mean, p.rstd, p.gamma, p.beta, p.slope, c);
   if (PHASE == 2) {
     const float* tot = p.ws + (size_t)p.nsplit * p.C * 4 + (size_t)c * 2;
-    dbeta_m = tot[0] * p.inv_count;
-    dgamma_m = tot[1] * p.inv_count;
+    k.dbeta_m = tot[0] * p.inv_count;
+    k.dgamma_m = tot[1] * p.inv_count;
   }
   float r[3] = {0.f, 0.f, 0.f};
   const bool has_skip = p.dskip != nullptr;
   auto elem = [&](float av, float dh, float ds) -> float {
     if (PHASE == 0) {
-      float g = dh * (av > 0.f ? 1.0f : sl);
+      const float g = prelu_skip_bwd(av, dh, ds, sl, al, has_skip);
       r[0] += dh * (av > 0.f ? 0.0f : av);
-      if (has_skip) {
-        g = fmaf(al, ds, g);
-        r[1] = fmaf(ds, av, r[1]);
-      }
+      if (has_skip) r[1] = fmaf(ds, av, r[1]);
       r[2] += g;
       return g;
     }
-    const float xh = (av - mu) * rs;
-    const float v = fmaf(av, sc, sh);
-    const float g = dh * (v > 0.f ? 1.0f : sl);
     if (PHASE == 1) {
+      float xh, v;
+      const float g = bn_prelu_gate(k, av, dh, xh, v);
       r[0] += dh * (v > 0.f ? 0.0f : v);
       r[1] += g;
       r[2] = fmaf(g, xh, r[2]);
       return 0.0f;
     }
-    const float d = ga * rs * (g - dbeta_m - xh * dgamma_m);
+    const float d = bn_prelu_bwd(k, av, dh);
     r[0] += d;
     return d;
   };
diff --git a/segan_pytorch_amd/csrc/segan_wgrad.hip b/segan_pytorch_amd/csrc/segan_wgrad.hip
--- a/segan_pytorch_amd/csrc/segan_wgrad.hip
+++ b/segan_pytorch_amd/csrc/segan_wgrad.hip
@@ -1,4 +1,5 @@
 #include "segan_conv_tile.h"
+#include "segan_act_bwd.h"
 
 
 template <int TK>
@@ -311,8 +312,17 @@
   }
 }
 
-template <int U, int RB, int NN, bool LO_ID, bool HI_ID>
-__global__ __launch_bounds__(256, RB >= 4 ? 1 : 2) void wgrad_edge_kernel(const WgradArgs a, int spw) {
+struct EdgeBnArgs {
+  BnBwdSrc s;
+  float* dbias;
+  float* dbias_slabs;
+};
+
+constexpr int wgrad_edge_occ(int RB, int NN, bool LO_BN) { return (RB >= 4 || (LO_BN && RB * NN >= 4)) ? 1 : 2; }
+
+template <int U, int RB, int NN, bool LO_ID, bool HI_ID, bool LO_BN = false>
+__global__ __launch_bounds__(256, wgrad_edge_occ(RB, NN, LO_BN)) void wgrad_edge_kernel(const WgradArgs a, int spw,
+                                                                          const EdgeBnArgs bn) {
   constexpr int S = 32 / U;
   constexpr int MB = RB <= 2 ? 64 : 128;
   constexpr int NIW = MB / 64;
@@ -325,7 +335,7 @@
   const int Ls = a.Ls, Lhi = a.Lhi;
   const int spb = Ls >> 5;
   const int nsteps = a.B * spb;
-  constexpr int DEPTH = RB * NN >= 4 ? 1 : 2;
+  constexpr int DEPTH = (LO_BN && RB >= 4) ? 0 : (RB * NN >= 4 || (LO_BN && RB >= 2)) ? 1 : 2;
   const int wg_beg = min(nsteps, (int)blockIdx.z * 4 * spw), wg_end = min(nsteps, wg_beg + 4 * spw);
   const int cnt = wg_end - wg_beg > wave ? (wg_end - wg_beg - wave + 3) / 4 : 0;
 
@@ -373,8 +383,25 @@
   constexpr int WLDS = NN * XL * 64 + RB * 1024;
   float* win = red + wave * WLDS;
   float* atile = win + NN * XL * 64;
+  constexpr int EXT = 4 * (WLDS > NBLK * 1024 ? WLDS : NBLK * 1024);
+  float* coef = red + EXT;
+  float* bsum = coef + 32 * RB * 8;
+  float rsum[RB][4];
+  if (LO_BN) {
+    if (tid < 32 * RB) {
+      const BnBwdCoef kc = bn_bwd_coef(bn.s, tid < a.M ? tid : 0);
+      *reinterpret_cast<f32x4*>(coef + 8 * tid) = f32x4{kc.mu, kc.rs, kc.sc, kc.sh};
+      *reinterpret_cast<f32x4*>(coef + 8 * tid + 4) = f32x4{kc.gr, kc.sl, kc.dbeta_m, kc.dgamma_m};
+    }
+#pragma unroll
+    for (int i = 0; i < RB; ++i)
+#pragma unroll
+      for (int q = 0; q < 4; ++q) rsum[i][q] = 0.0f;
+    __syncthreads();
+  }
   struct Regs {
     f32x4 A[RB][4];
+    f32x4 D[LO_BN ? RB : 1][4];
     float X[NN][XL];
     unsigned xok;
   };
@@ -387,7 +414,20 @@
     for (int i = 0; i < RB; ++i)
 #pragma unroll
       for (int q = 0; q < 4; ++q)
-        R.A[i][q] = *reinterpret_cast<const f32x4*>((cs1[i][q] ? sb1 : sb0) + crow[i][q]);
+        if (!LO_BN) R.A[i][q] = *reinterpret_cast<const f32x4*>((cs1[i][q] ? sb1 : sb0) + crow[i][q]);
+    if (LO_BN) {
+      const size_t so = (size_t)b * a.lo.C0 * Ls + t0;
+      const float* sa = a.lo.p0 + so;
+      const float* sd = bn.s.dh + so;
+#pragma unroll
+      for (int i = 0; i < RB; ++i)
+#pragma unroll
+        for (int q = 0; q < 4; ++q) {
+          const unsigned vo = (unsigned)crow[i][q] + 4u * lpc;
+          R.A[i][q] = *reinterpret_cast<const f32x4*>(sa + vo);
+          R.D[i][q] = *reinterpret_cast<const f32x4*>(sd + vo);
+        }
+    }
     R.xok = 0u;
     int off[XL];
 #pragma unroll
@@ -407,11 +447,34 @@
     }
   };
   auto compute = [&](Regs& R) {
-#pragma unroll
-    for (int i = 0; i < RB; ++i)
-#pragma unroll
-      for (int q = 0; q < 4; ++q)
-        *reinterpret_cast<f32x4*>(atile + (32 * i + 8 * q + lrow) * 32 + 4 * (lpc ^ lrow)) = R.A[i][q];
+    if (LO_BN) {
+#pragma unroll
+      for (int i = 0; i < RB; ++i)
+#pragma unroll
+        for (int q = 0; q < 4; ++q) {
+          const int row = 32 * i + 8 * q + lrow;
+          const f32x4 c0 = *reinterpret_cast<const f32x4*>(coef + 8 * row);
+          const f32x4 c1 = *reinterpret_cast<const f32x4*>(coef + 8 * row + 4);
+          BnBwdCoef kc;
+          kc.mu = c0[0]; kc.rs = c0[1]; kc.sc = c0[2]; kc.sh = c0[3];
+          kc.gr = c1[0]; kc.sl = c1[1]; kc.dbeta_m = c1[2]; kc.dgamma_m = c1[3];
+          f32x4 d4;
+#pragma unroll
+          for (int e = 0; e < 4; ++e) {
+            d4[e] = bn_prelu_bwd(kc, R.A[i][q][e], R.D[i][q][e]);
+            rsum[i][q] += d4[e];
+          }
+          *reinterpret_cast<f32x4*>(atile + row * 32 + 4 * (lpc ^ lrow)) = d4;
+        }
+      __builtin_amdgcn_sched_barrier(0);
+    }
+    if (!LO_BN) {
+#pragma unroll
+      for (int i = 0; i < RB; ++i)
+#pragma unroll
+        for (int q = 0; q < 4; ++q)
+          *reinterpret_cast<f32x4*>(atile + (32 * i + 8 * q + lrow) * 32 + 4 * (lpc ^ lrow)) = R.A[i][q];
+    }
     f32x4 Af[RB][4];
 #pragma unroll
     for (int i = 0; i < RB; ++i)
@@ -455,7 +518,13 @@
 
   if (cnt > 0) {
     auto stp = [&](int i) { return wg_beg + 4 * min(i, cnt - 1) + wave; };
-    if (DEPTH == 1) {
+    if (DEPTH == 0) {
+      Regs R0;
+      for (int i = 0; i < cnt; ++i) {
+        load(R0, stp(i));
+        compute(R0);
+      }
+    } else if (DEPTH == 1) {
       Regs R0, R1;
       load(R0, stp(0));
       for (int i = 0; i < cnt; i += 2) {
@@ -479,7 +548,24 @@
     }
   }
 
+  if (LO_BN && bn.dbias != nullptr) {
+#pragma unroll
+    for (int i = 0; i < RB; ++i)
+#pragma unroll
+      for (int q = 0; q < 4; ++q) {
+        float v = rsum[i][q];
+        v += __shfl_xor(v, 1, 64);
+        v += __shfl_xor(v, 2, 64);
+        v += __shfl_xor(v, 4, 64);
+        if (lpc == 0) bsum[wave * (32 * RB) + 32 * i + 8 * q + lrow] = v;
+      }
+  }
   __syncthreads();
+  if (LO_BN && bn.dbias != nullptr && tid < 32 * RB && tid < a.M) {
+    const float sb = ((bsum[tid] + bsum[32 * RB + tid]) + bsum[2 * 32 * RB + tid]) + bsum[3 * 32 * RB + tid];
+    if (bn.dbias_slabs) bn.dbias_slabs[(size_t)blockIdx.z * MB + tid] = sb;
+    else atomicAdd(bn.dbias + tid, sb);
+  }
 #pragma unroll
   for (int i = 0; i < RB; ++i)
 #pragma unroll
@@ -950,6 +1036,15 @@
   return SEGAN_OK;
 }
 
+__global__ void wgrad_edge_bias_reduce_kernel(const float* __restrict__ slabs, float* dbias, int nwg,
+                                              int MB, int M) {
+  const int m = threadIdx.x;
+  if (m >= M) return;
+  float s = 0.0f;
+  for (int z = 0; z < nwg; ++z) s += slabs[(size_t)z * MB + m];
+  dbias[m] += s;
+}
+
 static bool wgrad_edge_geometry_ok(const WgradArgs& a, int U) {
   if (a.Cv > 64 / U || a.N > 2) return false;
   if (a.Ls % 32 != 0) return false;
@@ -957,8 +1052,9 @@
   return true;
 }
 
-template <int U, int RB, int NN, bool LO_ID, bool HI_ID>
-static int launch_wgrad_edge_tile(WgradArgs& a, hipStream_t st, float* slabs, size_t slab_floats) {
+template <int U, int RB, int NN, bool LO_ID, bool HI_ID, bool LO_BN = false>
+static int launch_wgrad_edge_tile(WgradArgs& a, hipStream_t st, float* slabs, size_t slab_floats,
+                                  const EdgeBnArgs* ebn = nullptr) {
   constexpr int MB = RB <= 2 ? 64 : 128;
   if ((long)a.B * a.M * a.Ls >= (1L << 31) || (long)a.B * a.N * a.Lhi >= (1L << 31)) {
     segan_set_error("wgrad: operand exceeds the 2^31 element indexing limit");
@@ -967,7 +1063,7 @@
   if (int e = segan_src_defaults(&a.lo, st, "wgrad(lo)")) return e;
   if (int e = segan_src_defaults(&a.hi, st, "wgrad(hi)")) return e;
   const int nsteps = a.B * (a.Ls / 32);
-  constexpr int OCC = RB >= 4 ? 1 : 2;
+  constexpr int OCC = wgrad_edge_occ(RB, NN, LO_BN);
   int nwg = ceil_div(nsteps, 4 * 8);
   if (nwg > 256 * OCC) nwg = 256 * OCC;
   const int spw = ceil_div(nsteps, 4 * nwg);
@@ -975,24 +1071,34 @@
   a.w2_slabs = nullptr;
   if (nwg == 1) slabs = nullptr;
   if (slabs) {
-    if (slab_floats < (size_t)nwg * MB * 64) {
+    if (slab_floats < (size_t)nwg * MB * (LO_BN ? 65 : 64)) {
       segan_set_error("wgrad: deterministic mode needs %zu bytes of scratch for the partial tiles",
-                      (size_t)nwg * MB * 64 * sizeof(float));
+                      (size_t)nwg * MB * (LO_BN ? 65 : 64) * sizeof(float));
       return SEGAN_EINVAL;
     }
     a.w2_slabs = slabs;
+  }
+  EdgeBnArgs bn = {};
+  if (LO_BN) {
+    bn = *ebn;
+    bn.dbias_slabs = (slabs && bn.dbias) ? slabs + (size_t)nwg * MB * 64 : nullptr;
   }
   g_last_wgrad[0] = 4; g_last_wgrad[1] = 1; g_last_wgrad[2] = nwg; g_last_wgrad[3] = spw;
   g_last_wgrad[4] = 0; g_last_wgrad[5] = 0;
   constexpr int XL = (32 * (32 / U) + 32 + 63) / 64;
   const size_t lds_red = (size_t)4 * RB * NN * 1024 * sizeof(float);
   const size_t lds_win = (size_t)4 * (NN * XL * 64 + RB * 1024) * sizeof(float);
-  const size_t lds = lds_red > lds_win ? lds_red : lds_win;
-  auto kern = wgrad_edge_kernel<U, RB, NN, LO_ID, HI_ID>;
+  const size_t lds = (lds_red > lds_win ? lds_red : lds_win) + (LO_BN ? (size_t)32 * RB * 12 * sizeof(float) : 0);
+  auto kern = wgrad_edge_kernel<U, RB, NN, LO_ID, HI_ID, LO_BN>;
   static bool attr_done[16];
   allow_big_lds(kern, attr_done);
-  hipLaunchKernelGGL(kern, dim3(1, 1, nwg), dim3(256), lds, st, a, spw);
+  hipLaunchKernelGGL(kern, dim3(1, 1, nwg), dim3(256), lds, st, a, spw, bn);
   if (int e = segan_check_launch("wgrad_edge_kernel")) return e;
+  if (LO_BN && bn.dbias_slabs) {
+    hipLaunchKernelGGL(wgrad_edge_bias_reduce_kernel, dim3(1), dim3(128), 0, st, bn.dbias_slabs, bn.dbias,
+                       nwg, MB, a.M);
+    if (int e = segan_check_launch("wgrad_edge_bias_reduce_kernel")) return e;
+  }
   if (slabs) {
     int zstep = 1;
     if (nwg >= 128) {
@@ -1080,6 +1186,18 @@
     if (rc != SEGAN_EUNSUPPORTED) return rc;
   }
   return launch_wgrad_t<U>(a, st, slabs, slab_floats);
+}
+
+template <int U, bool HI_ID>
+static int launch_wgrad_edge_bn(WgradArgs& a, hipStream_t st, float* slabs, size_t slab_floats,
+                                const EdgeBnArgs& bn) {
+  if (a.N == 1) {
+    if (a.M <= 32) return launch_wgrad_edge_tile<U, 1, 1, true, HI_ID, true>(a, st, slabs, slab_floats, &bn);
+    if (a.M <= 64) return launch_wgrad_edge_tile<U, 2, 1, true, HI_ID, true>(a, st, slabs, slab_floats, &bn);
+    return launch_wgrad_edge_tile<U, 4, 1, true, HI_ID, true>(a, st, slabs, slab_floats, &bn);
+  }
+  if (a.M <= 32) return launch_wgrad_edge_tile<U, 1, 2, true, HI_ID, true>(a, st, slabs, slab_floats, &bn);
+  return launch_wgrad_edge_tile<U, 2, 2, true, HI_ID, true>(a, st, slabs, slab_floats, &bn);
 }
 
 extern "C" size_t segan_wgrad_scratch_bytes(int B, int M, int N, int Ls, int S, int precision,
@@ -1133,3 +1251,55 @@
     default: return launch_wgrad_fp32<32>(a, st, det, sc, scf);
   }
 }
+
+extern "C" int segan_wgrad_edge_bn(const float* a, const float* dh, const float* slope,
+                                   const float* bn_mean, const float* bn_rstd, const float* bn_gamma,
+                                   const float* bn_beta, const float* totals, double count_total,
+                                   const segan_src* hi, float* dw, float* dbias, int B, int M, int N,
+                                   int Ls, int K, int S, int padL, int mode, int roll, int flags,
+                                   void* scratch, size_t scratch_bytes, void* stream) {
+  SEGAN_REQUIRE(stride_ok(S), "wgrad_edge_bn: stride %d not in {1,2,4}", S);
+  SEGAN_REQUIRE(K >= 1 && K <= 32, "wgrad_edge_bn: kernel width %d not in [1,32]", K);
+  SEGAN_REQUIRE(B > 0 && N > 0 && M > 0 && Ls > 0, "wgrad_edge_bn: bad sizes");
+  SEGAN_REQUIRE(a && dh && bn_mean && bn_rstd && totals && dw, "wgrad_edge_bn: NULL pointer");
+  SEGAN_REQUIRE(count_total >= (double)B * Ls, "wgrad_edge_bn: bad element count");
+  SEGAN_REQUIRE(mode == SEGAN_PAD_REFLECT || mode == SEGAN_PAD_ZERO, "wgrad_edge_bn: bad pad mode");
+  if (int e = check_src(hi, N, "wgrad_edge_bn(hi)")) return e;
+  SEGAN_REQUIRE((((uintptr_t)a | (uintptr_t)dh) & 15) == 0,
+                "wgrad_edge_bn: a and dh must be 16-byte aligned");
+  const int L = S * Ls;
+  SEGAN_REQUIRE(roll > -L && roll < L, "wgrad_edge_bn: |roll| must be < L");
+  WgradArgs w = {};
+  w.lo.p0 = a; w.lo.p1 = nullptr; w.lo.C0 = M; w.lo.C1 = 0;
+  w.lo.scale = w.lo.shift = w.lo.slope = nullptr;
+  w.hi = *hi; w.dw = dw;
+  w.B = B; w.M = M; w.N = N; w.K = K; w.Ls = Ls; w.Lhi = L;
+  w.Cv = N * S; w.padL = padL; w.mode = mode; w.roll = roll;
+  w.Ctot = B * Ls;
+  const int U = 32 / S;
+  if (!wgrad_edge_geometry_ok(w, U)) {
+    segan_set_error("wgrad_edge_bn: not an edge geometry (N <= 2, Ls %% 32 == 0, M <= 128)");
+    return SEGAN_EUNSUPPORTED;
+  }
+  EdgeBnArgs bn = {};
+  bn.s.dh = dh; bn.s.mean = bn_mean; bn.s.rstd = bn_rstd; bn.s.gamma = bn_gamma; bn.s.beta = bn_beta;
+  bn.s.slope = slope; bn.s.totals = totals; bn.s.inv_count = (float)(1.0 / count_total);
+  bn.dbias = dbias;
+  hipStream_t st = (hipStream_t)stream;
+  float* slabs = nullptr;
+  size_t slab_floats = 0;
+  if (flags & SEGAN_WGRAD_DETERMINISTIC) {
+    SEGAN_REQUIRE(scratch != nullptr, "wgrad_edge_bn: deterministic mode needs scratch (segan_wgrad_scratch_bytes)");
+    slabs = (float*)scratch;
+    slab_floats = scratch_bytes / sizeof(float);
+  }
+  const bool hi_id = !w.hi.scale && !w.hi.shift && !w.hi.slope;
+#define EDGE_BN(UU) (hi_id ? launch_wgrad_edge_bn<UU, true>(w, st, slabs, slab_floats, bn) \
+                           : launch_wgrad_edge_bn<UU, false>(w, st, slabs, slab_floats, bn))
+  switch (S) {
+    case 4: return EDGE_BN(8);
+    case 2: return EDGE_BN(16);
+    default: return EDGE_BN(32);
+  }
+#undef EDGE_BN
+}
diff --git a/segan_pytorch_amd/distributed.py b/segan_pytorch_amd/distributed.py
--- a/segan_pytorch_amd/distributed.py
+++ b/segan_pytorch_amd/distributed.py
@@ -480,11 +480,16 @@
     return ops.bn_final(allp, gamma, beta, eps, momentum, running_mean, running_var)
 
 
-def act_bwd_bn_sync(a, dh, slope, bn, dslope=None, dgamma=None, dbeta=None, dbias=None):
+def act_bwd_bn_totals_sync(a, dh, slope, bn, dslope=None, dgamma=None, dbeta=None):
     totals, ws = ops.act_bwd_bn_reduce(a, dh, slope, bn, dslope, dgamma, dbeta)
     if _native_cur is not None:
         _native_cur.allreduce(totals, 1.0)
     else:
         dist.all_reduce(totals, op=dist.ReduceOp.SUM)
     count = float(a.shape[0]) * float(a.shape[2]) * world_size()
+    return totals, count, ws
+
+
+def act_bwd_bn_sync(a, dh, slope, bn, dslope=None, dgamma=None, dbeta=None, dbias=None):
+    totals, count, ws = act_bwd_bn_totals_sync(a, dh, slope, bn, dslope, dgamma, dbeta)
     return ops.act_bwd_bn_apply(a, dh, slope, bn, totals, count, dbias, ws)
diff --git a/segan_pytorch_amd/functional.py b/segan_pytorch_amd/functional.py
--- a/segan_pytorch_amd/functional.py
+++ b/segan_pytorch_amd/functional.py
@@ -70,6 +70,19 @@
         return sdist.act_bwd_bn_sync(a, dh, slope, bn, dslope, dgamma, dbeta, dbias)
     return ops.act_bwd(a, dh, slope=slope, bn=bn, dslope=dslope, dgamma=dgamma, dbeta=dbeta,
                        dbias=dbias)
+
+
+_FIRST_LAYER_ONLOAD = os.environ.get('SEGAN_FIRST_LAYER_ONLOAD', '1') != '0'
+
+
+def _first_layer_onload(disc_l, bn, c, N, need_w, need_x, need_b):
+    if not _FIRST_LAYER_ONLOAD or disc_l != 0 or bn is None or bn == 'eval' or need_w == need_x:
+        return False
+    if need_b and not need_w:
+        return False
+    if not c.is_cuda:
+        return False
+    return ops.edge_bn_ok(N, c.shape[1], c.shape[2], need_w)
 
 
 _WGRAD_OVERLAP = os.environ.get('SEGAN_WGRAD_OVERLAP', '0') == '1'
@@ -617,6 +630,32 @@
             if bn == 'eval':
                 raise RuntimeError('Discriminator backward in eval() mode with BatchNorm is not '
                                    'supported; call .train() (the reference never does this)')
+            need_w = W.needs_grad(blk.conv)
+            need_x = l == 0 and ctx.x_needs
+            need_b = blk.conv.bias is not None and blk.conv.bias.requires_grad
+            if _first_layer_onload(l, bn, cs[l], srcs[l].C, need_w, need_x, need_b):
+                slope = blk.act.weight
+                from . import distributed as sdist
+                if sdist.sync_bn_enabled():
+                    totals, count, _ws_red = sdist.act_bwd_bn_totals_sync(cs[l], dh, slope, bn, _gb(slope),
+                                                                         _gb(bn[2]), _gb(bn[3]))
+                else:
+                    totals, _ws_red = ops.act_bwd_bn_reduce(cs[l], dh, slope, bn, _gb(slope), _gb(bn[2]),
+                                                            _gb(bn[3]))
+                    count = cs[l].shape[0] * cs[l].shape[2]
+                padL = ops.conv_pad(K, S)[0]
+                if need_w:
+                    with _SideStream(cs[l], dh, totals, srcs[l]):
+                        gw = W.grad_target(blk.conv)
+                        ops.wgrad_edge_bn(cs[l], dh, slope, bn, totals, count, srcs[l], gw, K, S, padL,
+                                          PAD_REFLECT, roll=ctx.rolls[l], dbias=_gb(blk.conv.bias))
+                        W.finish(blk.conv, gw)
+                        _ready(blk)
+                else:
+                    _ready(blk)
+                    dx = ops.conv1d_dgrad_edge_bn(cs[l], dh, slope, bn, totals, count, w, srcs[l].L, S,
+                                                  roll=ctx.rolls[l], padL=padL)
+                continue
             if bn is not None:
                 dc = _act_bwd_bn(cs[l], dh, blk.act.weight, bn, _gb(blk.act.weight), _gb(bn[2]),
                                  _gb(bn[3]), _gb(blk.conv.bias))
diff --git a/segan_pytorch_amd/ops.py b/segan_pytorch_amd/ops.py
--- a/segan_pytorch_amd/ops.py
+++ b/segan_pytorch_amd/ops.py
@@ -413,6 +413,65 @@
                           pad_mode, roll, PREC_FP32, flags,
                           ctypes.c_void_p(scratch.data_ptr()) if scratch is not None else None, nbytes,
                           _stream()), 'wgrad')
+
+
+def edge_bn_ok(N, M, Ls, wgrad_side):
+    if _precision != PREC_FP32 or N > 2 or Ls % 32 != 0 or M > 128:
+        return False
+    return not (wgrad_side and N > 1 and M > 64)
+
+
+def wgrad_edge_bn(a, dh, slope, bn, totals, count_total, hi, dw, K, S, padL, pad_mode, roll=0,
+                  dbias=None):
+    _chk(a, 'a', 3)
+    _chk(dh, 'dh', 3)
+    _chk(dw, 'dw', 3)
+    if dh.shape != a.shape:
+        raise ValueError('wgrad_edge_bn: dh {} vs a {}'.format(tuple(dh.shape), tuple(a.shape)))
+    B, M, Ls = a.shape
+    N = hi.C
+    if tuple(dw.shape) != (M, N, K):
+        raise ValueError('wgrad_edge_bn: dw {} != ({}, {}, {})'.format(tuple(dw.shape), M, N, K))
+    if hi.B != B or Ls * S != hi.L:
+        raise ValueError('wgrad_edge_bn: a [{}x{}] / hi [{}x{}] inconsistent for stride {}'.format(
+            B, Ls, hi.B, hi.L, S))
+    mean, rstd, gamma, beta = bn
+    ch = hi.c_struct()
+    lib = _lib.load()
+    flags = 1 if _deterministic else 0
+    scratch, nbytes = None, 0
+    if flags:
+        nbytes = lib.segan_wgrad_scratch_bytes(B, M, N, Ls, S, PREC_FP32, flags)
+        scratch = _stream_scratch(nbytes, dw.device)
+    check(lib.segan_wgrad_edge_bn(_ptr(a), _ptr(dh), _ptr(slope), _ptr(mean), _ptr(rstd), _ptr(gamma),
+                                  _ptr(beta), _ptr(totals), float(count_total), ctypes.byref(ch),
+                                  _ptr(dw), _ptr(dbias), B, M, N, Ls, K, S, padL, pad_mode, roll, flags,
+                                  ctypes.c_void_p(scratch.data_ptr()) if scratch is not None else None,
+                                  nbytes, _stream()), 'wgrad_edge_bn')
+
+
+def conv1d_dgrad_edge_bn(a, dh, slope, bn, totals, count_total, w, L, S, roll=0, padL=None):
+    _chk(a, 'a', 3)
+    _chk(dh, 'dh', 3)
+    _chk(w, 'weight', 3)
+    if dh.shape != a.shape:
+        raise ValueError('conv1d_dgrad_edge_bn: dh {} vs a {}'.format(tuple(dh.shape), tuple(a.shape)))
+    M, N, K = w.shape
+    B = a.shape[0]
+    if a.shape[1] != M or a.shape[2] * S != L:
+        raise ValueError('conv1d_dgrad_edge_bn: a {} inconsistent with weight {} / L {}'.format(
+            tuple(a.shape), tuple(w.shape), L))
+    if padL is None:
+        padL = conv_pad(K, S)[0]
+    mean, rstd, gamma, beta = bn
+    dx = torch.empty((B, N, L), device=a.device, dtype=torch.float32)
+    halo = torch.empty((B * N * max(K - 1, 1),), device=a.device, dtype=torch.float32)
+    check(_lib.load().segan_conv1d_dgrad_edge_bn(_ptr(a), _ptr(dh), _ptr(slope), _ptr(mean), _ptr(rstd),
+                                                 _ptr(gamma), _ptr(beta), _ptr(totals),
+                                                 float(count_total), _ptr(w.detach()), _ptr(dx),
+                                                 _ptr(halo), B, N, M, L, K, S, padL, roll, _stream()),
+          'conv1d_dgrad_edge_bn')
+    return dx
 
 
 def deconv1d_fwd(src, w, bias, S, act=ACT_NONE, pack=None):
```
